# r-barnes/richdem

Measured on NVIDIA H100. Metric: Priority-Flood fill + D8 flow accumulation throughput, higher is better.
Workload: dtype f32

## Files before the change

richdem_b200/csrc/fill.cu:

```cuda
#include "common.cuh"

#include <chrono>

namespace rdb {

namespace {

#ifndef RDB_TX
#define RDB_TX 64
#endif
#ifndef RDB_TY
#define RDB_TY 64
#endif
#ifndef RDB_FILL_THREADS
#define RDB_FILL_THREADS 128
#endif
#ifndef RDB_FILL_MIN_CTAS
#define RDB_FILL_MIN_CTAS 6
#endif
constexpr int TX = RDB_TX;
constexpr int TY = RDB_TY;
constexpr int BXN = TX / 4;
constexpr int BYN = TY / 4;
constexpr int PADL = 4;
constexpr int SP = TX + 2 * PADL;
constexpr int SROWS = TY + 2;
constexpr int FILL_THREADS = RDB_FILL_THREADS;
constexpr int FILL_MIN_CTAS = RDB_FILL_MIN_CTAS;
static_assert(BYN <= 16 && BXN * BYN <= 256 && TX % 4 == 0 && TY % 4 == 0, "tile shape");
constexpr uint32_t W_TILE_BYTES = SP * SROWS * 4;
constexpr uint32_t Z_TILE_BYTES = TX * TY * 4;

struct RoundCtl {
  int count;
  int take;
};

struct FillDev {
  RoundCtl ctl[3];
  RoundCtl proc[3];
  unsigned long long visits;
  unsigned long long iters;
  unsigned long long block_updates;
  unsigned long long warp_updates;
  unsigned long long idle_visits;
  unsigned long long iter_hist[8];
  int edge_changed;
  int zmin_ord, zmax_ord;
  unsigned long long deferred;
  unsigned long long live_rounds;
  float level, step, step_min, level_max;
  int target, ordered;
  int ndefer[3];
};

struct FillArgs {
  const float *Z;
  int zpitch, zox, zoy, zext;
  const float *coarse;
  int Wc, pool, yoff;
  int *staged;
  float *Wp;
  int pitch;
  int W, H;
  int tilesX, tilesY;
  int *list0, *list1;
  int *stamp;
  int *sides;
  int *keys;
  float level;
  int *plist;
  int use_proc;
  FillDev *dev;
  int round;
  int max_iters;
  int use_tma;
  int profile;
  int *dirty;
};

__device__ __forceinline__ uint32_t smem_u32(const void *p) {
  return (uint32_t)__cvta_generic_to_shared(p);
}
__device__ __forceinline__ void mbar_init(unsigned long long *bar, int count) {
  asm volatile("mbarrier.init.shared::cta.b64 [%0], %1;" ::"r"(smem_u32(bar)), "r"(count) : "memory");
}
__device__ __forceinline__ void mbar_arrive_expect_tx(unsigned long long *bar, uint32_t bytes) {
  asm volatile("mbarrier.arrive.expect_tx.shared::cta.b64 _, [%0], %1;" ::"r"(smem_u32(bar)),
               "r"(bytes)
               : "memory");
}
__device__ __forceinline__ void mbar_wait(unsigned long long *bar, uint32_t parity) {
  uint32_t ok;
  const uint32_t addr = smem_u32(bar);
  do {
    asm volatile(
        "{\n"
        "  .reg .pred p;\n"
        "  mbarrier.try_wait.parity.shared::cta.b64 p, [%1], %2;\n"
        "  selp.u32 %0, 1, 0, p;\n"
        "}\n"
        : "=r"(ok)
        : "r"(addr), "r"(parity)
        : "memory");
  } while (!ok);
}
__device__ __forceinline__ void tma_load_2d(void *smem_dst, const CUtensorMap *map, int c0, int c1,
                                            unsigned long long *bar) {
  asm volatile(
      "cp.async.bulk.tensor.2d.shared::cluster.global.mbarrier::complete_tx::bytes [%0], [%1, {%2, %3}], [%4];"
      ::"r"(smem_u32(smem_dst)),
      "l"((unsigned long long)map), "r"(c0), "r"(c1), "r"(smem_u32(bar))
      : "memory");
}
__device__ __forceinline__ void fence_proxy_async() {
  asm volatile("fence.proxy.async.shared::cta;" ::: "memory");
}

constexpr int NBLK = BXN * BYN;
constexpr int MKP = BXN + 2;
constexpr int NWARP = FILL_THREADS / 32;
constexpr int SEG = ((NBLK + NWARP - 1) / NWARP + 31) / 32 * 32;
enum : int { SIDE_N = 1, SIDE_S = 2, SIDE_W = 4, SIDE_E = 8, SIDE_NW = 16, SIDE_NE = 32, SIDE_SW = 64,
             SIDE_SE = 128, SIDE_FULL = 256 };

__host__ __device__ __forceinline__ int f2ord(float f) {
  int b;
  memcpy(&b, &f, 4);
  return b >= 0 ? b : (b ^ 0x7fffffff);
}
__host__ __device__ __forceinline__ float ord2f(int o) {
  const int b = o >= 0 ? o : (o ^ 0x7fffffff);
  float f;
  memcpy(&f, &b, 4);
  return f;
}
constexpr int ORD_POS_INF = 0x7f800000;

__device__ __forceinline__ void enqueue_tile(const FillArgs &a, RoundCtl *next, int *list_next, int t,
                                             int stampval, int side_bits, int key_ord) {
  atomicOr(&a.sides[(stampval & 1) * a.tilesX * a.tilesY + t], side_bits);
  atomicMin(&a.keys[(stampval & 1) * a.tilesX * a.tilesY + t], key_ord);
  if (atomicExch(&a.stamp[t], stampval) != stampval) {
    const int idx = atomicAdd(&next->count, 1);
    list_next[idx] = t;
  }
}

__device__ __forceinline__ float min3f(float a, float b, float c) { return fminf(fminf(a, b), c); }

constexpr bool DRAIN_SWEEPS = TX == 64 && TY == 64 && FILL_THREADS == 128;

template <bool TOPO4>
__device__ __forceinline__ void fill_drain_sweeps(float *sW, const float *sZ, int y0, int H, int *sFlags, int *sKey) {
  const unsigned FULL = 0xffffffffu;
  const int tid = threadIdx.x, lane = tid & 31, wrp = tid >> 5;
  const int x = 32 * (wrp & 1) + lane;
  const bool down = wrp < 2;
  const int dy = down ? 1 : -1;
  const bool ecol = x < 4 || x >= TX - 4;
  unsigned long long rows = 0;
  float kmin = __int_as_float(0x7f800000);
  int y = down ? 0 : TY - 1;
  float p = sW[(y - dy + 1) * SP + PADL + x];
#pragma unroll 1
  for (int half = 0; half < 2; half++) {
#pragma unroll 8
    for (int s = 0; s < TY / 2; s++, y += dy) {
      const float zz = sZ[y * TX + x];
      float *cell = &sW[(y + 1) * SP + PADL + x];
      const float w = *cell;
      float m = p;
      if (!TOPO4) {
        float pl = __shfl_up_sync(FULL, p, 1), pr = __shfl_down_sync(FULL, p, 1);
        const float *prow = &sW[(y - dy + 1) * SP + PADL + x];
        if (lane == 0) pl = prow[-1];
        if (lane == 31) pr = prow[1];
        m = min3f(pl, p, pr);
      }
      const float nw = fminf(w, fmaxf(zz, m));
      p = w;
      if (nw < w) {
        *cell = nw;
        p = nw;
        rows |= 1ull << y;
        if (ecol || y < 4 || y >= TY - 4) kmin = fminf(kmin, nw);
      }
    }
    __syncthreads();
  }
  int f = 0;
#pragma unroll
  for (int by = 0; by < BYN; by++)
    if ((rows >> (4 * by)) & 0xFull) f |= 1 << (12 + by);
  if (rows & 1ull) f |= SIDE_N;
  if (rows >> (TY - 1)) f |= SIDE_S;
  if (x == 0 && rows) f |= SIDE_W | (rows & 1ull ? SIDE_NW : 0) | (rows >> (TY - 1) ? SIDE_SW : 0);
  if (x == TX - 1 && rows) f |= SIDE_E | (rows & 1ull ? SIDE_NE : 0) | (rows >> (TY - 1) ? SIDE_SE : 0);
  const int j1 = 1 - y0, j2 = (H - 2) - y0;
  if (j1 >= 0 && j1 < TY && ((rows >> j1) & 1ull)) f |= 1 << 9;
  if (j2 >= 0 && j2 < TY && ((rows >> j2) & 1ull)) f |= 1 << 10;
#pragma unroll
  for (int o = 16; o > 0; o >>= 1) {
    f |= __shfl_xor_sync(FULL, f, o);
    kmin = fminf(kmin, __shfl_xor_sync(FULL, kmin, o));
  }
  if (lane == 0 && f) {
    atomicOr(sFlags, f);
    if (f & 0xFF) atomicMin(sKey, f2ord(kmin));
  }
}

template <int STEP, bool TOPO4 = false, bool STAGE = false>
__global__ void __launch_bounds__(FILL_THREADS, FILL_MIN_CTAS)
    fill_sweep_kernel(const __grid_constant__ CUtensorMap mapW, const __grid_constant__ CUtensorMap mapZ,
                      const FillArgs a) {
  __shared__ __align__(128) float sW[SROWS * SP];
  __shared__ __align__(128) float sZ[TY * TX];
  __shared__ __align__(8) unsigned long long mbar;
  __shared__ unsigned char sMark[MKP * (BYN + 2)];
  __shared__ unsigned char sList[2][NWARP][SEG];
  __shared__ __align__(16) int sCnt[2][NWARP];
  __shared__ int sTile;
  __shared__ int sFlags;
  __shared__ int sKey;
  __shared__ int sProf[2];
  __shared__ int sNbDone;

  const int tid = threadIdx.x;
  const int r = a.round;
  RoundCtl *cur = &a.dev->ctl[r % 3];
  RoundCtl *next = &a.dev->ctl[(r + 1) % 3];
  const int *list_cur = (r & 1) ? a.list1 : a.list0;
  int *list_next = (r & 1) ? a.list0 : a.list1;
  const int ntiles = a.tilesX * a.tilesY;
  if (a.use_proc) {
    cur = &a.dev->proc[r % 3];
    list_cur = a.plist;
  }
  const int n = cur->count;

  if (blockIdx.x == 0 && tid == 0) {
    RoundCtl *z = &a.dev->ctl[(r + 2) % 3];
    z->count = 0;
    z->take = 0;
    RoundCtl *zp = &a.dev->proc[(r + 1) % 3];
    zp->count = 0;
    zp->take = 0;
    if (n > 0) {
      atomicAdd(&a.dev->visits, (unsigned long long)n);
      a.dev->live_rounds++;
    }
  }
  if (n == 0) return;

  if (tid == 0) {
    mbar_init(&mbar, 1);
    asm volatile("fence.mbarrier_init.release.cluster;" ::: "memory");
  }
  uint32_t phase = 0;
  const int max_iters = a.max_iters;

  for (;;) {
    if (tid == 0) sTile = atomicAdd(&cur->take, 1);
    for (int k = tid; k < MKP * (BYN + 2); k += FILL_THREADS) sMark[k] = 0;
    __syncthreads();
    const int li = sTile;
    if (li >= n) break;
    const int t = list_cur[li];
    const int tyT = t / a.tilesX, txT = t - tyT * a.tilesX;
    const int x0 = txT * TX, y0 = tyT * TY;

    constexpr bool stage = STAGE;
    if (tid == 0) {
      sFlags = 0;
      sKey = ORD_POS_INF;
      sProf[0] = sProf[1] = 0;
      if (stage) {
        int nb = 0;
        for (int dy = -1; dy <= 1; dy++)
          for (int dx = -1; dx <= 1; dx++) {
            const int ty = tyT + dy, tx = txT + dx;
            if ((dx | dy) && ty >= 0 && ty < a.tilesY && tx >= 0 && tx < a.tilesX &&
                *reinterpret_cast<volatile int *>(&a.staged[ty * a.tilesX + tx]))
              nb |= 1 << ((dy + 1) * 3 + dx + 1);
          }
        __threadfence();
        sNbDone = nb;
      }
    }
    if (a.use_tma) {
      if (tid == 0) {
        fence_proxy_async();
        mbar_arrive_expect_tx(&mbar, (stage ? 0u : W_TILE_BYTES) + Z_TILE_BYTES);
        if (!stage) tma_load_2d(sW, &mapW, x0, y0, &mbar);
        tma_load_2d(sZ, &mapZ, x0 + a.zox, y0 + a.zoy, &mbar);
      }
    } else {
      if (!stage) {
        for (int k = tid; k < SROWS * (SP / 4); k += FILL_THREADS) {
          const int rr = k / (SP / 4), cc = k - rr * (SP / 4);
          reinterpret_cast<float4 *>(sW)[k] =
              __ldcg(reinterpret_cast<const float4 *>(a.Wp + (size_t)(y0 + rr) * a.pitch + x0) + cc);
        }
      }
      const float inf = __int_as_float(0x7f800000);
      for (int k = tid; k < TY * (TX / 4); k += FILL_THREADS) {
        const int rr = k / (TX / 4), cc = k - rr * (TX / 4);
        reinterpret_cast<float4 *>(sZ)[k] =
            a.zext && (y0 + rr >= a.H || x0 + 4 * cc >= a.W)
                ? make_float4(inf, inf, inf, inf)
                : __ldg(reinterpret_cast<const float4 *>(a.Z + (size_t)(y0 + a.zoy + rr) * a.zpitch + x0 + a.zox) + cc);
      }
    }
    int sides = a.sides[(r & 1) * ntiles + t];
    __syncthreads();
    if (tid == 0) {
      a.sides[(r & 1) * ntiles + t] = 0;
      a.keys[(r & 1) * ntiles + t] = ORD_POS_INF;
    }
    if (stage) {
      const float inf = __int_as_float(0x7f800000);
      const int nbdone = sNbDone;
      constexpr int C4N = SP / 4, RSTEP = FILL_THREADS / C4N;
      static_assert(RSTEP >= 1, "a CTA covers one row of the window");
      if (tid < RSTEP * C4N) {
        const int c4 = 4 * (tid % C4N);
        int rr = tid / C4N;
        const int dx = c4 < PADL ? -1 : (c4 >= PADL + TX ? 1 : 0);
        const int xb = x0 + c4 - PADL;
        const int cx = xb >= 0 ? xb / a.pool : 0, rx = xb - cx * a.pool;
        const int yy = y0 + rr - 1 + a.yoff;
        int cy = (yy + a.pool) / a.pool - 1, ry = yy - cy * a.pool;
        const int dq = RSTEP / a.pool, dr = RSTEP - dq * a.pool;
        for (; rr < SROWS; rr += RSTEP) {
          const int dy = rr == 0 ? -1 : (rr == SROWS - 1 ? 1 : 0);
          float4 v4;
          if ((nbdone >> ((dy + 1) * 3 + dx + 1)) & 1) {
            v4 = __ldcg(reinterpret_cast<const float4 *>(a.Wp + (size_t)(y0 + rr) * a.pitch + x0 + c4));
          } else {
            const int y = y0 + rr - 1;
            float v[4] = {inf, inf, inf, inf};
            if (y >= 0 && y < a.H) {
              const float *crow = a.coarse + (size_t)cy * a.Wc;
              const float *zrow = a.Z + (size_t)(y + a.zoy) * a.zpitch + a.zox;
              const bool brow = y == 0 || y == a.H - 1;
              const float c0 = (a.pool & 3) == 0 && xb >= 0 && xb < a.W ? __ldg(crow + cx) : inf;
              int cc = cx, rc = rx;
#pragma unroll
              for (int j = 0; j < 4; j++) {
                const int x = xb + j;
                if (j > 0 && ++rc == a.pool) {
                  rc = 0;
                  cc++;
                }
                if (x >= 0 && x < a.W)
                  v[j] = brow || x == 0 || x == a.W - 1 ? __ldg(zrow + x) : (a.pool & 3) == 0 ? c0 : __ldg(crow + cc);
              }
            }
            v4 = make_float4(v[0], v[1], v[2], v[3]);
          }
          *reinterpret_cast<float4 *>(&sW[rr * SP + c4]) = v4;
          cy += dq;
          ry += dr;
          if (ry >= a.pool) {
            ry -= a.pool;
            cy++;
          }
        }
      }
    }
#include "fill_relax_body.inc"

    if (f) {
      atomicOr(&sFlags, f);
      if (f & 0xFF) atomicMin(&sKey, f2ord(kmin));
    }
    __syncthreads();
    const int fl = sFlags;
    const int rowch = (fl >> 12) & 0xFFFF;
    const int rowout = stage ? (1 << BYN) - 1 : rowch;
    if (rowout) {
      for (int k = tid; k < TY * (TX / 4); k += FILL_THREADS) {
        const int rr = k / (TX / 4), cc = k % (TX / 4);
        if (rowout & (1 << (rr >> 2))) {
          const float4 val = *reinterpret_cast<const float4 *>(&sW[(rr + 1) * SP + PADL + 4 * cc]);
          __stcg(reinterpret_cast<float4 *>(a.Wp + (size_t)(y0 + 1 + rr) * a.pitch + (x0 + PADL)) + cc, val);
        }
      }
    }
    if (stage) {
      __syncthreads();
      if (tid == 0) {
        __threadfence();
        atomicExch(&a.staged[t], 1);
      }
    }
    if (rowch) {
      if (tid < 8) {
        const int sv = r + 1;
        const bool n_ok = tyT > 0, s_ok = tyT < a.tilesY - 1, w_ok = txT > 0, e_ok = txT < a.tilesX - 1;
        int nb = -1, bits = 0;
        switch (tid) {
          case 0: if ((fl & SIDE_N) && n_ok) { nb = t - a.tilesX; bits = SIDE_S; } break;
          case 1: if ((fl & SIDE_S) && s_ok) { nb = t + a.tilesX; bits = SIDE_N; } break;
          case 2: if ((fl & SIDE_W) && w_ok) { nb = t - 1; bits = SIDE_E; } break;
          case 3: if ((fl & SIDE_E) && e_ok) { nb = t + 1; bits = SIDE_W; } break;
          case 4: if ((fl & SIDE_NW) && n_ok && w_ok) { nb = t - a.tilesX - 1; bits = SIDE_SE; } break;
          case 5: if ((fl & SIDE_NE) && n_ok && e_ok) { nb = t - a.tilesX + 1; bits = SIDE_SW; } break;
          case 6: if ((fl & SIDE_SW) && s_ok && w_ok) { nb = t + a.tilesX - 1; bits = SIDE_NE; } break;
          default: if ((fl & SIDE_SE) && s_ok && e_ok) { nb = t + a.tilesX + 1; bits = SIDE_NW; } break;
        }
        if (nb >= 0) enqueue_tile(a, next, list_next, nb, sv, bits, sKey);
        if (tid == 0 && (fl & (3 << 9))) atomicOr(&a.dev->edge_changed, (fl >> 9) & 3);
        if (tid == 0 && a.dirty) a.dirty[t] = 1;
      }
    }
    if (tid == 0) {
      if (again) enqueue_tile(a, next, list_next, t, r + 1, SIDE_FULL, f2ord(-__int_as_float(0x7f800000)));
      atomicAdd(&a.dev->iters, (unsigned long long)iters);
      if (a.profile) {
        if (!rowch) atomicAdd(&a.dev->idle_visits, 1ull);
        atomicAdd(&a.dev->block_updates, (unsigned long long)sProf[0]);
        atomicAdd(&a.dev->warp_updates, (unsigned long long)sProf[1]);
        const int hb = iters <= 1 ? 0 : iters <= 2 ? 1 : iters <= 4 ? 2 : iters <= 8 ? 3 : iters <= 16 ? 4 : iters <= 32 ? 5 : iters <= 64 ? 6 : 7;
        atomicAdd(&a.dev->iter_hist[hb], 1ull);
      }
    }
  }
}

__global__ void __launch_bounds__(256) fill_admit_kernel(const FillArgs a) {
  const int r = a.round;
  const RoundCtl *cur = &a.dev->ctl[r % 3];
  RoundCtl *next = &a.dev->ctl[(r + 1) % 3];
  RoundCtl *proc = &a.dev->proc[r % 3];
  const int *list_cur = (r & 1) ? a.list1 : a.list0;
  int *list_next = (r & 1) ? a.list0 : a.list1;
  const int n = cur->count;
  const int ntiles = a.tilesX * a.tilesY;
  const float level = a.level;
  int nd = 0;
  for (int i = blockIdx.x * blockDim.x + threadIdx.x; i < n; i += gridDim.x * blockDim.x) {
    const int t = list_cur[i];
    const int kord = a.keys[(r & 1) * ntiles + t];
    if (ord2f(kord) <= level) {
      a.plist[atomicAdd(&proc->count, 1)] = t;
    } else {
      int bits = a.sides[(r & 1) * ntiles + t];
      if (bits == 0) bits = SIDE_FULL;
      a.sides[(r & 1) * ntiles + t] = 0;
      a.keys[(r & 1) * ntiles + t] = ORD_POS_INF;
      enqueue_tile(a, next, list_next, t, r + 1, bits, kord);
      nd++;
    }
  }
  for (int o = 16; o > 0; o >>= 1) nd += __shfl_xor_sync(0xffffffffu, nd, o);
  if ((threadIdx.x & 31) == 0 && nd) atomicAdd(&a.dev->ndefer[r % 3], nd);
}

__global__ void __launch_bounds__(256) fill_seed_kernel(const FillArgs a, const int *__restrict__ tiles, int n) {
  const int i = blockIdx.x * blockDim.x + threadIdx.x;
  if (i >= n) return;
  const int r = a.round;
  RoundCtl *cur = &a.dev->ctl[r % 3];
  int *list_cur = (r & 1) ? a.list1 : a.list0;
  enqueue_tile(a, cur, list_cur, tiles[i], r, SIDE_FULL, f2ord(-__int_as_float(0x7f800000)));
}

__global__ void __launch_bounds__(256) fill_seed_flags_kernel(const FillArgs a, const int *__restrict__ flag, int ntiles,
                                                               int *count) {
  const int t = blockIdx.x * blockDim.x + threadIdx.x;
  if (t >= ntiles || !flag[t]) return;
  const int r = a.round;
  RoundCtl *cur = &a.dev->ctl[r % 3];
  int *list_cur = (r & 1) ? a.list1 : a.list0;
  enqueue_tile(a, cur, list_cur, t, r, SIDE_FULL, f2ord(-__int_as_float(0x7f800000)));
  if (count) atomicAdd(count, 1);
}

__global__ void __launch_bounds__(256) fill_ghost_update_kernel(float *Wp, float *Zp, int pitch, int W, int H, int y,
                                                                 const float *__restrict__ row, int *tile_flag, int tilesX,
                                                                 int *lowered) {
  const int x = blockIdx.x * blockDim.x + threadIdx.x;
  if (x >= W) return;
  const size_t o = (size_t)(y + 1) * pitch + x + PADL;
  const float v = row[x];
  if (v < Wp[o]) {
    Wp[o] = v;
    Zp[o] = v;
    *lowered = 1;
    const int ya = y > 0 ? y - 1 : 0, yb = y < H - 1 ? y + 1 : H - 1, xa = x > 0 ? x - 1 : 0, xb = x < W - 1 ? x + 1 : W - 1;
    const int ty0 = ya / TY, ty1 = yb / TY, tx0 = xa / TX, tx1 = xb / TX;
    tile_flag[ty0 * tilesX + tx0] = 1;
    if (tx1 != tx0) tile_flag[ty0 * tilesX + tx1] = 1;
    if (ty1 != ty0) {
      tile_flag[ty1 * tilesX + tx0] = 1;
      if (tx1 != tx0) tile_flag[ty1 * tilesX + tx1] = 1;
    }
  }
}

__global__ void __launch_bounds__(256) fill_lift_row_kernel(float *row, int W, const float *__restrict__ coarse_row, int k) {
  const int x = blockIdx.x * blockDim.x + threadIdx.x;
  if (x < W) row[x] = coarse_row[x / k];
}

template <bool LIFT>
__global__ void fill_init_kernel(const float *__restrict__ dem, float *__restrict__ Zp,
                                 float *__restrict__ Wp, int W, int H, int pitch, int rows, FillDev *dev,
                                 const float *__restrict__ coarse, int Wc, int pool, int yoff) {
  const int px4 = (blockIdx.x * blockDim.x + threadIdx.x) * 4;
  const float inf = __int_as_float(0x7f800000);
  float lo = inf, hi = -inf;
  for (int py = blockIdx.y; py < rows && px4 < pitch; py += gridDim.y) {
    float zv[4], wv[4];
    const int y = py - 1;
#pragma unroll
    for (int k = 0; k < 4; k++) {
      const int x = px4 + k - PADL;
      float zz = inf, ww = inf;
      if (x >= 0 && x < W && y >= 0 && y < H) {
        zz = dem[(size_t)y * W + x];
        const bool border = (x == 0) | (y == 0) | (x == W - 1) | (y == H - 1);
        ww = border ? zz : (LIFT ? __ldg(coarse + (size_t)((y + yoff) / pool) * Wc + x / pool) : inf);
        if (zz < inf && zz > -inf) {
          lo = fminf(lo, zz);
          hi = fmaxf(hi, zz);
        }
      }
      zv[k] = zz;
      wv[k] = ww;
    }
    const size_t o = (size_t)py * pitch + px4;
    if (Zp) *reinterpret_cast<float4 *>(Zp + o) = make_float4(zv[0], zv[1], zv[2], zv[3]);
    *reinterpret_cast<float4 *>(Wp + o) = make_float4(wv[0], wv[1], wv[2], wv[3]);
  }
  for (int o = 16; o > 0; o >>= 1) {
    lo = fminf(lo, __shfl_xor_sync(0xffffffffu, lo, o));
    hi = fmaxf(hi, __shfl_xor_sync(0xffffffffu, hi, o));
  }
  __shared__ float slo[4], shi[4];
  if ((threadIdx.x & 31) == 0) {
    slo[threadIdx.x >> 5] = lo;
    shi[threadIdx.x >> 5] = hi;
  }
  __syncthreads();
  if (threadIdx.x == 0) {
    lo = fminf(fminf(slo[0], slo[1]), fminf(slo[2], slo[3]));
    hi = fmaxf(fmaxf(shi[0], shi[1]), fmaxf(shi[2], shi[3]));
    if (lo <= hi) {
      atomicMin(&dev->zmin_ord, f2ord(lo));
      atomicMax(&dev->zmax_ord, f2ord(hi));
    }
  }
}

__global__ void __launch_bounds__(256) fill_frame_kernel(float *__restrict__ Wp, int pitch, int rows) {
  const int i = blockIdx.x * blockDim.x + threadIdx.x;
  const float inf = __int_as_float(0x7f800000);
  if (i < pitch) {
    Wp[i] = inf;
    Wp[(size_t)(rows - 1) * pitch + i] = inf;
  }
  if (i < rows) {
#pragma unroll
    for (int j = 0; j < PADL; j++) {
      Wp[(size_t)i * pitch + j] = inf;
      Wp[(size_t)i * pitch + pitch - PADL + j] = inf;
    }
  }
}

constexpr int HIST_BINS = 1024;
__global__ void __launch_bounds__(256) fill_hist_kernel(const float *__restrict__ Z, int zpitch, int ncols, int nrows,
                                                         int row_stride, float zmin, float inv_range, unsigned int *hist) {
  __shared__ unsigned int sh[HIST_BINS];
  for (int k = threadIdx.x; k < HIST_BINS; k += blockDim.x) sh[k] = 0;
  __syncthreads();
  const int row = blockIdx.x * row_stride;
  if (row < nrows) {
    for (int x = threadIdx.x; x < ncols; x += blockDim.x) {
      const float zv = Z[(size_t)row * zpitch + x];
      if (zv < __int_as_float(0x7f800000) && zv > -__int_as_float(0x7f800000)) {
        int b = (int)((zv - zmin) * inv_range * HIST_BINS);
        b = b < 0 ? 0 : (b >= HIST_BINS ? HIST_BINS - 1 : b);
        atomicAdd(&sh[b], 1u);
      }
    }
  }
  __syncthreads();
  for (int k = threadIdx.x; k < HIST_BINS; k += blockDim.x)
    if (sh[k]) atomicAdd(&hist[k], sh[k]);
}

__global__ void __launch_bounds__(128) dist_pad_init_kernel(const uint8_t *__restrict__ open, int open_bit,
                                                             const float *__restrict__ winit, float *__restrict__ Zp,
                                                             float *__restrict__ Wp, int W, int H, int pitch, int rows,
                                                             int ghost_top, int ghost_bottom, int *tile_flag, int tilesX) {
  const int px = blockIdx.x * blockDim.x + threadIdx.x;
  if (px >= pitch) return;
  const float inf = __int_as_float(0x7f800000);
  for (int py = blockIdx.y; py < rows; py += gridDim.y) {
    const int x = px - PADL, y = py - 1;
    float zz = inf, ww = inf;
    if (x >= 0 && x < W && y >= 0 && y < H) {
      const size_t i = (size_t)y * W + x;
      if (!((ghost_top && y == 0) || (ghost_bottom && y == H - 1))) {
        if (open[i] & open_bit) zz = 0.0f;
        ww = winit[i];
        if (ww < inf) {
          const int ya = y > 0 ? y - 1 : 0, yb = y < H - 1 ? y + 1 : H - 1, xa = x > 0 ? x - 1 : 0, xb = x < W - 1 ? x + 1 : W - 1;
          const int ty0 = ya / TY, ty1 = yb / TY, tx0 = xa / TX, tx1 = xb / TX;
          tile_flag[ty0 * tilesX + tx0] = 1;
          if (tx1 != tx0) tile_flag[ty0 * tilesX + tx1] = 1;
          if (ty1 != ty0) {
            tile_flag[ty1 * tilesX + tx0] = 1;
            if (tx1 != tx0) tile_flag[ty1 * tilesX + tx1] = 1;
          }
        }
      }
    }
    Zp[(size_t)py * pitch + px] = zz;
    Wp[(size_t)py * pitch + px] = ww;
  }
}

__global__ void fill_i32_kernel(int *p, int v, int n) {
  const int i = blockIdx.x * blockDim.x + threadIdx.x;
  if (i < n) p[i] = v;
}

__global__ void __launch_bounds__(256) fill_maxpool_kernel(const float *__restrict__ src, int W, int H, int yoff, float *dst, int Wc,
                                                            int Hc, int k, int combine) {
  const int bx = blockIdx.x * blockDim.x + threadIdx.x;
  if (bx >= Wc) return;
  const int by_lo = yoff / k, by_hi = (yoff + H - 1) / k;
  for (int by = by_lo + blockIdx.y; by <= by_hi && by < Hc; by += gridDim.y) {
    float m = -__int_as_float(0x7f800000);
    const bool vec = (k & 3) == 0 && (W & 3) == 0 && bx * k + k <= W && ((uintptr_t)src & 15) == 0;
    for (int j = 0; j < k; j++) {
      const int y = by * k + j - yoff;
      if (y < 0) continue;
      if (y >= H) break;
      if (vec) {
        const float4 *row = reinterpret_cast<const float4 *>(src + (size_t)y * W + bx * k);
        for (int i = 0; i < k / 4; i++) {
          const float4 q = __ldg(row + i);
          m = fmaxf(fmaxf(m, fmaxf(q.x, q.y)), fmaxf(q.z, q.w));
        }
      } else {
        for (int i = 0; i < k; i++) {
          const int x = bx * k + i;
          if (x < W) m = fmaxf(m, __ldg(src + (size_t)y * W + x));
        }
      }
    }
    float *o = dst + (size_t)by * Wc + bx;
    *o = combine ? fmaxf(*o, m) : m;
  }
}

__global__ void __launch_bounds__(256) fill_restrict_kernel(const float *__restrict__ Wp, int pitch, int W, int H,
                                                             float *Wc, int cpitch, int Wcw, int Hc, int k,
                                                             const int *__restrict__ dirty, int tilesX, int *ctile_flag,
                                                             int ctilesX) {
  const int bx = blockIdx.x * blockDim.x + threadIdx.x;
  if (bx >= Wcw) return;
  for (int by = blockIdx.y; by < Hc; by += gridDim.y) {
    if (dirty && !dirty[((by * k) / TY) * tilesX + (bx * k) / TX]) continue;
    float m = -__int_as_float(0x7f800000);
    if ((k & 3) == 0 && bx * k + k <= W && by * k + k <= H) {
      for (int j = 0; j < k; j++) {
        const float4 *row = reinterpret_cast<const float4 *>(Wp + (size_t)(by * k + j + 1) * pitch + bx * k + PADL);
        for (int i = 0; i < k / 4; i++) {
          const float4 q = __ldcg(row + i);
          m = fmaxf(fmaxf(m, fmaxf(q.x, q.y)), fmaxf(q.z, q.w));
        }
      }
    } else {
      for (int j = 0; j < k; j++) {
        const int y = by * k + j;
        if (y >= H) break;
        for (int i = 0; i < k; i++) {
          const int x = bx * k + i;
          if (x < W) m = fmaxf(m, __ldcg(Wp + (size_t)(y + 1) * pitch + x + PADL));
        }
      }
    }
    float *o = Wc + (size_t)(by + 1) * cpitch + bx + PADL;
    if (m < *o && bx > 0 && by > 0 && bx < Wcw - 1 && by < Hc - 1) {
      *o = m;
      const int ty0 = (by - 1) / TY, ty1 = (by + 1) / TY, tx0 = (bx - 1) / TX, tx1 = (bx + 1) / TX;
      ctile_flag[ty0 * ctilesX + tx0] = 1;
      if (tx1 != tx0) ctile_flag[ty0 * ctilesX + tx1] = 1;
      if (ty1 != ty0) {
        ctile_flag[ty1 * ctilesX + tx0] = 1;
        if (tx1 != tx0) ctile_flag[ty1 * ctilesX + tx1] = 1;
      }
    }
  }
}

__global__ void __launch_bounds__(256) fill_blockmax_kernel(const float *__restrict__ Wp, int pitch, int W, int y_lo, int y_hi,
                                                             int yoff, float *out, int Wcw, int Hc, int k,
                                                             const int *__restrict__ dirty, int tilesX) {
  const int bx = blockIdx.x * blockDim.x + threadIdx.x;
  if (bx >= Wcw) return;
  const int by_lo = (yoff + y_lo) / k, by_hi = (yoff + y_hi - 1) / k;
  for (int by = by_lo + blockIdx.y; by <= by_hi && by < Hc; by += gridDim.y) {
    if (dirty) {
      int l0 = by * k - yoff, l1 = l0 + k - 1;
      l0 = l0 < y_lo ? y_lo : l0;
      l1 = l1 >= y_hi ? y_hi - 1 : l1;
      const int tx = (bx * k) / TX;
      if (!dirty[(l0 / TY) * tilesX + tx] && !dirty[(l1 / TY) * tilesX + tx]) {
        out[(size_t)by * Wcw + bx] = __int_as_float(0x7f800000);
        continue;
      }
    }
    float m = -__int_as_float(0x7f800000);
    for (int j = 0; j < k; j++) {
      const int y = by * k + j - yoff;
      if (y < y_lo) continue;
      if (y >= y_hi) break;
      for (int i = 0; i < k; i++) {
        const int x = bx * k + i;
        if (x < W) m = fmaxf(m, __ldcg(Wp + (size_t)(y + 1) * pitch + x + PADL));
      }
    }
    float *o = out + (size_t)by * Wcw + bx;
    *o = fmaxf(*o, m);
  }
}

__global__ void __launch_bounds__(256) fill_prolong_kernel(float *Wp, int pitch, int W, int H, const float *__restrict__ Wc,
                                                            int cpitch, int coff_x, int coff_y, int k, int *tile_flag,
                                                            int tilesX, int yoff, const int *__restrict__ cdirty,
                                                            int ctilesX) {
  const int t = blockIdx.x;
  const int tyT = t / tilesX, txT = t - tyT * tilesX;
  const int x0 = txT * TX, y0 = tyT * TY;
  if (cdirty) {
    const int cx0 = (x0 / k) / TX, cx1 = ((x0 + TX - 1) / k) / TX;
    const int cy0 = ((y0 + yoff) / k) / TY, cy1 = ((y0 + TY - 1 + yoff) / k) / TY;
    bool any = false;
    for (int cy = cy0; cy <= cy1; cy++)
      for (int cx = cx0; cx <= cx1; cx++) any |= cdirty[cy * ctilesX + cx] != 0;
    if (!any) return;
  }
  bool lowered = false, lo_n = false, lo_s = false, lo_w = false, lo_e = false;
  for (int g = threadIdx.x; g < TX * TY / 4; g += blockDim.x) {
    const int ly = g / (TX / 4), lx4 = (g - ly * (TX / 4)) * 4;
    const int y = y0 + ly;
    if (y < 1 || y >= H - 1) continue;
    float4 *wp4 = reinterpret_cast<float4 *>(Wp + (size_t)(y + 1) * pitch + x0 + lx4 + PADL);
    const float4 w4 = *wp4;
    float wv[4] = {w4.x, w4.y, w4.z, w4.w};
    const float *crow = Wc + (size_t)((y + yoff) / k + coff_y) * cpitch + coff_x;
    bool any = false;
#pragma unroll
    for (int j = 0; j < 4; j++) {
      const int lx = lx4 + j, x = x0 + lx;
      if (x < 1 || x >= W - 1) continue;
      const float l = __ldg(crow + x / k);
      if (l < wv[j]) {
        wv[j] = l;
        any = true;
        lo_w |= lx == 0;
        lo_e |= lx == TX - 1;
      }
    }
    if (any) {
      *wp4 = make_float4(wv[0], wv[1], wv[2], wv[3]);
      lowered = true;
      lo_n |= ly == 0;
      lo_s |= ly == TY - 1;
    }
  }
  if (lowered) {
    const int tilesY = (H + TY - 1) / TY;
    tile_flag[t] = 1;
    const bool n_ok = tyT > 0, s_ok = tyT < tilesY - 1, w_ok = txT > 0, e_ok = txT < tilesX - 1;
    if (lo_n && n_ok) tile_flag[t - tilesX] = 1;
    if (lo_s && s_ok) tile_flag[t + tilesX] = 1;
    if (lo_w && w_ok) tile_flag[t - 1] = 1;
    if (lo_e && e_ok) tile_flag[t + 1] = 1;
    if (lo_n && lo_w && n_ok && w_ok) tile_flag[t - tilesX - 1] = 1;
    if (lo_n && lo_e && n_ok && e_ok) tile_flag[t - tilesX + 1] = 1;
    if (lo_s && lo_w && s_ok && w_ok) tile_flag[t + tilesX - 1] = 1;
    if (lo_s && lo_e && s_ok && e_ok) tile_flag[t + tilesX + 1] = 1;
  }
}

__global__ void __launch_bounds__(256) fill_finish_x4_kernel(const float *__restrict__ Wp, float *__restrict__ out, int W,
                                                              int H, int pitch) {
  const int x4 = (blockIdx.x * blockDim.x + threadIdx.x) * 4;
  if (x4 >= W) return;
  for (int y = blockIdx.y; y < H; y += gridDim.y) {
    const float4 v = __ldcs(reinterpret_cast<const float4 *>(Wp + (size_t)(y + 1) * pitch + x4 + PADL));
    __stcs(reinterpret_cast<float4 *>(out + (size_t)y * W + x4), v);
  }
}

__global__ void fill_finish_kernel(const float *__restrict__ Wp, float *__restrict__ out, int W, int H,
                                   int pitch) {
  const int x = blockIdx.x * blockDim.x + threadIdx.x;
  if (x >= W) return;
  for (int y = blockIdx.y; y < H; y += gridDim.y) out[(size_t)y * W + x] = Wp[(size_t)(y + 1) * pitch + x + PADL];
}

typedef CUresult (*EncodeTiledFn)(CUtensorMap *, CUtensorMapDataType, cuuint32_t, void *, const cuuint64_t *,
                                  const cuuint64_t *, const cuuint32_t *, const cuuint32_t *,
                                  CUtensorMapInterleave, CUtensorMapSwizzle, CUtensorMapL2promotion,
                                  CUtensorMapFloatOOBfill);

EncodeTiledFn get_encode_fn() {
  static EncodeTiledFn fn = nullptr;
  if (!fn) {
    void *p = nullptr;
    cudaDriverEntryPointQueryResult q;
    RDB_CK(cudaGetDriverEntryPoint("cuTensorMapEncodeTiled", &p, cudaEnableDefault, &q));
    if (!p || q != cudaDriverEntryPointSuccess) fail("cuTensorMapEncodeTiled not available from the driver");
    fn = (EncodeTiledFn)p;
  }
  return fn;
}

CUtensorMap make_map(float *base, int pitch, int rows, int boxw, int boxh) {
  CUtensorMap m;
  const cuuint64_t gdim[2] = {(cuuint64_t)pitch, (cuuint64_t)rows};
  const cuuint64_t gstride[1] = {(cuuint64_t)pitch * 4};
  const cuuint32_t box[2] = {(cuuint32_t)boxw, (cuuint32_t)boxh};
  const cuuint32_t estr[2] = {1, 1};
  CUresult rc = get_encode_fn()(&m, CU_TENSOR_MAP_DATA_TYPE_FLOAT32, 2, base, gdim, gstride, box, estr,
                                CU_TENSOR_MAP_INTERLEAVE_NONE, CU_TENSOR_MAP_SWIZZLE_NONE,
                                CU_TENSOR_MAP_L2_PROMOTION_L2_128B, CU_TENSOR_MAP_FLOAT_OOB_FILL_NONE);
  if (rc != CUDA_SUCCESS) fail("cuTensorMapEncodeTiled failed with CUresult %d", (int)rc);
  return m;
}

}

struct FillState {
  int W = 0, H = 0, pitch = 0, rows = 0, tilesX = 0, tilesY = 0;
  DevBuf<float> Zp, Wp;
  DevBuf<int> list0, list1, plist, stamp, sides, keys;
  DevBuf<int> dirty, tflag;
  DevBuf<int> staged;
  float zmin = 0.f, zmax = 0.f;
  bool first_run = true;
  bool ordered = false;
  int step_mode = 0;
  bool topo4 = false;
  std::vector<float> levels;
  DevBuf<FillDev> dev;
  CUtensorMap mapW, mapZ;
  int round = 0;
  int grid = 0;
  int64_t rounds_run = 0;
  int64_t live_rounds = 0;
  int64_t visits_seen = 0;
  bool still_active = false;
  int64_t sched_round = 0;

  const float *zext = nullptr;
  const float *stage_coarse = nullptr;
  int stage_wc = 0, stage_k = 1, stage_yoff = 0;

  void begin(const float *d_dem, int w, int h, const float *d_coarse = nullptr, int coarse_w = 0, int coarse_k = 0,
             int coarse_yoff = 0, bool dem_stays = false) {
    Ctx &c = ctx();
    W = w;
    H = h;
    tilesX = (w + TX - 1) / TX;
    tilesY = (h + TY - 1) / TY;
    pitch = tilesX * TX + 2 * PADL;
    rows = tilesY * TY + 2;
    const size_t np = (size_t)pitch * rows;
    zext = dem_stays && c.params.fill_external_z != 0 && (w & 3) == 0 && ((uintptr_t)d_dem & 15) == 0 ? d_dem : nullptr;
    stage_coarse = zext && d_coarse ? d_coarse : nullptr;
    stage_wc = coarse_w;
    stage_k = coarse_k;
    stage_yoff = coarse_yoff;
    if (zext) Zp.reset();
    else Zp.alloc(np);
    Wp.alloc(np);
    const size_t nt = (size_t)tilesX * tilesY;
    list0.alloc(nt);
    list1.alloc(nt);
    plist.alloc(nt);
    stamp.alloc(nt);
    sides.alloc(2 * nt);
    keys.alloc(2 * nt);
    dev.alloc(1);
    RDB_CK(cudaMemsetAsync(stamp.p, 0, nt * sizeof(int), c.stream));
    RDB_CK(cudaMemsetAsync(sides.p, 0, 2 * nt * sizeof(int), c.stream));
    if (stage_coarse) {
      staged.alloc(nt);
      RDB_CK(cudaMemsetAsync(staged.p, 0, nt * sizeof(int), c.stream));
    }
    {
      FillDev h0;
      memset(&h0, 0, sizeof(h0));
      h0.zmin_ord = ORD_POS_INF;
      h0.zmax_ord = f2ord(-__builtin_inff());
      memcpy(c.pinned, &h0, sizeof(h0));
      RDB_CK(cudaMemcpyAsync(dev.p, c.pinned, sizeof(FillDev), cudaMemcpyHostToDevice, c.stream));
    }
    {
      const int n2 = (int)(2 * nt);
      fill_i32_kernel<<<(n2 + 255) / 256, 256, 0, c.stream>>>(keys.p, ORD_POS_INF, n2);
      dim3 blk(128), grd((pitch / 4 + 127) / 128, rows < 2048 ? rows : 2048);
      if (stage_coarse) {
        const int n = pitch > rows ? pitch : rows;
        fill_frame_kernel<<<(n + 255) / 256, 256, 0, c.stream>>>(Wp.p, pitch, rows);
      } else if (d_coarse) {
        fill_init_kernel<true><<<grd, blk, 0, c.stream>>>(d_dem, Zp.p, Wp.p, W, H, pitch, rows, dev.p, d_coarse, coarse_w, coarse_k,
                                                         coarse_yoff);
      } else {
        fill_init_kernel<false><<<grd, blk, 0, c.stream>>>(d_dem, Zp.p, Wp.p, W, H, pitch, rows, dev.p, nullptr, 0, 1, 0);
      }
      RDB_CK(cudaGetLastError());
      count_launch(2);
      zmin = zmax = 0.f;
      if (!d_coarse) {
        FillDev *hd = (FillDev *)c.pinned;
        RDB_CK(cudaMemcpyAsync(hd, dev.p, sizeof(FillDev), cudaMemcpyDeviceToHost, c.stream));
        RDB_CK(cudaStreamSynchronize(c.stream));
        zmin = ord2f(hd->zmin_ord);
        zmax = ord2f(hd->zmax_ord);
        if (!(zmin <= zmax)) zmin = zmax = 0.f;
      }
      ordered = c.params.fill_ordered != 0 && zmax > zmin && !d_coarse;
      levels.clear();
      if (ordered) {
        int64_t R = c.params.fill_order_rounds;
        if (R <= 0) R = (int64_t)(0.8 * (tilesX > tilesY ? tilesX : tilesY));
        if (R < 8) {
          ordered = false;
        } else {
          DevBuf<unsigned int> hist(HIST_BINS);
          RDB_CK(cudaMemsetAsync(hist.p, 0, HIST_BINS * sizeof(unsigned int), c.stream));
          const int stride = rows > 4096 ? 16 : (rows > 512 ? 4 : 1);
          const int nb = (rows - 2 + stride - 1) / stride;
          if (zext)
            fill_hist_kernel<<<nb, 256, 0, c.stream>>>(zext, W, W, H, stride, zmin, 1.0f / (zmax - zmin), hist.p);
          else
            fill_hist_kernel<<<nb, 256, 0, c.stream>>>(Zp.p + pitch, pitch, pitch, rows - 1, stride, zmin, 1.0f / (zmax - zmin),
                                                       hist.p);
          RDB_CK(cudaGetLastError());
          count_launch();
          unsigned int *hh = (unsigned int *)c.pinned;
          RDB_CK(cudaMemcpyAsync(hh, hist.p, HIST_BINS * sizeof(unsigned int), cudaMemcpyDeviceToHost, c.stream));
          RDB_CK(cudaStreamSynchronize(c.stream));
          double total = 0;
          for (int k = 0; k < HIST_BINS; k++) total += hh[k];
          levels.resize((size_t)R);
          double cum = 0;
          int bin = 0;
          for (int64_t k = 0; k < R; k++) {
            const double want = total * (double)(k + 1) / (double)R;
            while (bin < HIST_BINS - 1 && cum + hh[bin] < want) cum += hh[bin++];
            levels[(size_t)k] = zmin + (zmax - zmin) * (float)(bin + 1) / (float)HIST_BINS;
          }
        }
      }
    }
    mapW = make_map(Wp.p, pitch, rows, SP, SROWS);
    mapZ = zext ? make_map(const_cast<float *>(zext), W, H, TX, TY) : make_map(Zp.p, pitch, rows, TX, TY);
    int per_sm = 0;
    RDB_CK(cudaOccupancyMaxActiveBlocksPerMultiprocessor(&per_sm, fill_sweep_kernel<0>, FILL_THREADS, 0));
    if (per_sm < 1) per_sm = 1;
    grid = c.num_sms * per_sm;
    round = 1;
    std::vector<int> init;
    for (int ty = 0; ty < tilesY; ty++)
      for (int tx = 0; tx < tilesX; tx++)
        if (d_coarse || ty == 0 || tx == 0 || ty == tilesY - 1 || tx == tilesX - 1) init.push_back(ty * tilesX + tx);
    seed_worklist(init);
  }

  void begin_dist(const uint8_t *d_open, int open_bit, const float *d_winit, int w, int h, int ghost_top = 0,
                  int ghost_bottom = 0) {
    Ctx &c = ctx();
    step_mode = 1;
    W = w;
    H = h;
    tilesX = (w + TX - 1) / TX;
    tilesY = (h + TY - 1) / TY;
    pitch = tilesX * TX + 2 * PADL;
    rows = tilesY * TY + 2;
    const size_t np = (size_t)pitch * rows;
    Zp.alloc(np);
    Wp.alloc(np);
    const size_t nt = (size_t)tilesX * tilesY;
    list0.alloc(nt);
    list1.alloc(nt);
    plist.alloc(nt);
    stamp.alloc(nt);
    sides.alloc(2 * nt);
    keys.alloc(2 * nt);
    dev.alloc(1);
    RDB_CK(cudaMemsetAsync(stamp.p, 0, nt * sizeof(int), c.stream));
    RDB_CK(cudaMemsetAsync(sides.p, 0, 2 * nt * sizeof(int), c.stream));
    RDB_CK(cudaMemsetAsync(dev.p, 0, sizeof(FillDev), c.stream));
    const int n2 = (int)(2 * nt);
    fill_i32_kernel<<<(n2 + 255) / 256, 256, 0, c.stream>>>(keys.p, ORD_POS_INF, n2);
    dim3 blk(128), grd((pitch + 127) / 128, rows < 2048 ? rows : 2048);
    clear_flags();
    dist_pad_init_kernel<<<grd, blk, 0, c.stream>>>(d_open, open_bit, d_winit, Zp.p, Wp.p, W, H, pitch, rows, ghost_top,
                                                    ghost_bottom, tflag.p, tilesX);
    RDB_CK(cudaGetLastError());
    count_launch(2);
    ordered = false;
    mapW = make_map(Wp.p, pitch, rows, SP, SROWS);
    mapZ = make_map(Zp.p, pitch, rows, TX, TY);
    int per_sm = 0;
    RDB_CK(cudaOccupancyMaxActiveBlocksPerMultiprocessor(&per_sm, fill_sweep_kernel<1>, FILL_THREADS, 0));
    if (per_sm < 1) per_sm = 1;
    grid = c.num_sms * per_sm;
    round = 1;
    seed_from_flags();
  }

  void seed_worklist(const std::vector<int> &tiles) {
    Ctx &c = ctx();
    if (tiles.empty()) return;
    DevBuf<int> d(tiles.size());
    RDB_CK(cudaMemcpyAsync(d.p, tiles.data(), tiles.size() * sizeof(int), cudaMemcpyHostToDevice, c.stream));
    FillArgs a = make_args();
    a.round = round;
    fill_seed_kernel<<<(unsigned)((tiles.size() + 255) / 256), 256, 0, c.stream>>>(a, d.p, (int)tiles.size());
    RDB_CK(cudaGetLastError());
    count_launch();
    RDB_CK(cudaStreamSynchronize(c.stream));
  }

  FillArgs make_args() {
    Ctx &c = ctx();
    FillArgs a;
    memset(&a, 0, sizeof(a));
    if (zext) {
      a.Z = zext;
      a.zpitch = W;
      a.zext = 1;
    } else {
      a.Z = Zp.p;
      a.zpitch = pitch;
      a.zox = PADL;
      a.zoy = 1;
    }
    a.Wc = stage_wc;
    a.pool = stage_k;
    a.yoff = stage_yoff;
    a.staged = staged.p;
    a.Wp = Wp.p;
    a.pitch = pitch;
    a.W = W;
    a.H = H;
    a.tilesX = tilesX;
    a.tilesY = tilesY;
    a.list0 = list0.p;
    a.list1 = list1.p;
    a.stamp = stamp.p;
    a.sides = sides.p;
    a.keys = keys.p;
    a.plist = plist.p;
    a.dev = dev.p;
    a.max_iters = (int)c.params.fill_max_iters;
    a.use_tma = (int)c.params.fill_use_tma;
    a.profile = (int)c.params.fill_profile;
    a.level = __builtin_inff();
    a.dirty = dirty.p;
    return a;
  }

  bool timed = true;
  int batch_edge = 0;
  void launch_batch(int per_sync) {
    Ctx &c = ctx();
    FillArgs a = make_args();
    if (timed) RDB_CK(cudaEventRecord(c.evk0, c.stream));
    for (int k = 0; k < per_sync; k++) {
      a.round = round;
      if (ordered && sched_round < (int64_t)levels.size()) {
        a.level = levels[(size_t)sched_round];
        a.use_proc = 1;
        fill_admit_kernel<<<c.num_sms * 2, 256, 0, c.stream>>>(a);
        c.stats.kernel_launches++;
      } else {
        a.level = __builtin_inff();
        a.use_proc = 0;
      }
      sched_round++;
      a.coarse = round == 1 ? stage_coarse : nullptr;
      if (step_mode) fill_sweep_kernel<1><<<grid, FILL_THREADS, 0, c.stream>>>(mapW, mapZ, a);
      else if (a.coarse && topo4) fill_sweep_kernel<0, true, true><<<grid, FILL_THREADS, 0, c.stream>>>(mapW, mapZ, a);
      else if (a.coarse) fill_sweep_kernel<0, false, true><<<grid, FILL_THREADS, 0, c.stream>>>(mapW, mapZ, a);
      else if (topo4) fill_sweep_kernel<0, true><<<grid, FILL_THREADS, 0, c.stream>>>(mapW, mapZ, a);
      else fill_sweep_kernel<0><<<grid, FILL_THREADS, 0, c.stream>>>(mapW, mapZ, a);
      round++;
    }
    if (timed) RDB_CK(cudaEventRecord(c.evk1, c.stream));
    RDB_CK(cudaGetLastError());
    RDB_CK(cudaMemcpyAsync(c.pinned, dev.p, sizeof(FillDev), cudaMemcpyDeviceToHost, c.stream));
    c.stats.kernel_launches += per_sync;
    rounds_run += per_sync;
    if (round > (1 << 30)) fail("fill: round counter overflow");
  }
  bool collect() {
    Ctx &c = ctx();
    RDB_CK(cudaStreamSynchronize(c.stream));
    if (timed) {
      float t = 0;
      RDB_CK(cudaEventElapsedTime(&t, c.evk0, c.evk1));
      c.stats.ms_main_kernel += t;
    }
    const FillDev *hd = (const FillDev *)c.pinned;
    still_active = hd->ctl[round % 3].count != 0;
    if (!still_active) first_run = false;
    live_rounds = (int64_t)hd->live_rounds;
    visits_seen = (int64_t)hd->visits;
    iters_seen = (int64_t)hd->iters;
    batch_edge = hd->edge_changed;
    return still_active;
  }
  int64_t iters_seen = 0;

  int run(int64_t max_rounds = 0) {
    Ctx &c = ctx();
    int64_t rounds_this_call = 0;
    int per_sync = (int)(c.params.fill_rounds_per_sync > 0 ? c.params.fill_rounds_per_sync : 16);
    if (max_rounds > 0 && max_rounds < per_sync) per_sync = (int)max_rounds;
    RDB_CK(cudaMemsetAsync(&dev.p->edge_changed, 0, sizeof(int), c.stream));
    for (;;) {
      launch_batch(per_sync);
      collect();
      rounds_this_call += per_sync;
      if (!still_active) break;
      if (max_rounds > 0 && rounds_this_call >= max_rounds) break;
    }
    const FillDev *hd = (const FillDev *)c.pinned;
    c.stats.fill_rounds = live_rounds;
    c.stats.fill_tile_visits = visits_seen;
    c.stats.fill_tile_iters = iters_seen;
    c.stats.fill_tile_cells = TX * TY;
    if (c.params.fill_profile) {
      fprintf(stderr, "[fill profile] deferred=%llu visits=%llu iters=%llu block_updates=%llu (%.1f%% of 256/iter) warp_updates=%llu (%.1f%% of 8/iter) idle_visits=%llu hist(1,2,3-4,5-8,9-16,17-32,33-64,65+)=",
              hd->deferred, hd->visits, hd->iters, hd->block_updates, 100.0 * hd->block_updates / (256.0 * hd->iters + 1),
              hd->warp_updates, 100.0 * hd->warp_updates / (8.0 * hd->iters + 1), hd->idle_visits);
      for (int k = 0; k < 8; k++) fprintf(stderr, "%llu ", hd->iter_hist[k]);
      fprintf(stderr, "\n");
    }
    return batch_edge | (still_active ? 4 : 0);
  }

  void track_dirty() {
    Ctx &c = ctx();
    const size_t nt = (size_t)tilesX * tilesY;
    dirty.alloc(nt);
    RDB_CK(cudaMemsetAsync(dirty.p, 0, nt * sizeof(int), c.stream));
  }
  void clear_dirty() {
    if (dirty.p) RDB_CK(cudaMemsetAsync(dirty.p, 0, (size_t)tilesX * tilesY * sizeof(int), ctx().stream));
  }
  void seed_from_flags(int *d_count = nullptr) {
    Ctx &c = ctx();
    const int nt = tilesX * tilesY;
    FillArgs a = make_args();
    a.round = round;
    fill_seed_flags_kernel<<<(nt + 255) / 256, 256, 0, c.stream>>>(a, tflag.p, nt, d_count);
    RDB_CK(cudaGetLastError());
    count_launch();
  }
  void clear_flags() {
    const size_t nt = (size_t)tilesX * tilesY;
    if (!tflag.p) tflag.alloc(nt);
    RDB_CK(cudaMemsetAsync(tflag.p, 0, nt * sizeof(int), ctx().stream));
  }
  void restrict_into(FillState &cs, int k) {
    Ctx &c = ctx();
    cs.clear_flags();
    const bool selective = dirty.p && TX % k == 0 && TY % k == 0;
    dim3 blk(256), grd((unsigned)((cs.W + 255) / 256), (unsigned)(cs.H < 4096 ? cs.H : 4096));
    fill_restrict_kernel<<<grd, blk, 0, c.stream>>>(Wp.p, pitch, W, H, cs.Wp.p, cs.pitch, cs.W, cs.H, k,
                                                    selective ? dirty.p : nullptr, tilesX, cs.tflag.p, cs.tilesX);
    RDB_CK(cudaGetLastError());
    count_launch();
    cs.seed_from_flags();
    clear_dirty();
  }
  void blockmax_into(float *d_out, int wc, int hc, int k, int yoff, int y_lo, int y_hi, bool selective = false) {
    Ctx &c = ctx();
    dim3 blk(256), grd((unsigned)((wc + 255) / 256), (unsigned)((y_hi - y_lo) / k + 2 < 4096 ? (y_hi - y_lo) / k + 2 : 4096));
    const bool sel = selective && dirty.p && TX % k == 0;
    fill_blockmax_kernel<<<grd, blk, 0, c.stream>>>(Wp.p, pitch, W, y_lo, y_hi, yoff, d_out, wc, hc, k, sel ? dirty.p : nullptr, tilesX);
    RDB_CK(cudaGetLastError());
    count_launch();
    if (sel) clear_dirty();
  }
  void prolong_from(const float *d_wc, int cpitch, int coff_x, int coff_y, int k, int yoff = 0, const int *cdirty = nullptr,
                    int ctilesX = 0, int *d_count = nullptr) {
    Ctx &c = ctx();
    clear_flags();
    const int nt = tilesX * tilesY;
    fill_prolong_kernel<<<nt, 256, 0, c.stream>>>(Wp.p, pitch, W, H, d_wc, cpitch, coff_x, coff_y, k, tflag.p, tilesX, yoff,
                                                  cdirty, ctilesX);
    RDB_CK(cudaGetLastError());
    count_launch();
    seed_from_flags(d_count);
  }
  void prolong_from_level(FillState &cs, int k, int yoff = 0, int *d_count = nullptr) {
    prolong_from(cs.Wp.p, cs.pitch, PADL, 1, k, yoff, cs.dirty.p, cs.tilesX, d_count);
    cs.clear_dirty();
  }
  void ghost_update(int y, const float *d_row, int *d_lowered) {
    Ctx &c = ctx();
    clear_flags();
    fill_ghost_update_kernel<<<(W + 255) / 256, 256, 0, c.stream>>>(Wp.p, Zp.p, pitch, W, H, y, d_row, tflag.p, tilesX, d_lowered);
    RDB_CK(cudaGetLastError());
    count_launch();
    seed_from_flags();
  }

  void read_row(int y, float *d_row) {
    if (y < 0 || y >= H) fail("fill_read_row: row %d out of range", y);
    RDB_CK(cudaMemcpyAsync(d_row, Wp.p + (size_t)(y + 1) * pitch + PADL, (size_t)W * 4,
                           cudaMemcpyDeviceToDevice, ctx().stream));
  }

  void update_row(int y, const float *d_row) {
    if (y != 0 && y != H - 1) fail("fill_update_row: only boundary rows (0, height-1) can be replaced");
    Ctx &c = ctx();
    const size_t o = (size_t)(y + 1) * pitch + PADL;
    RDB_CK(cudaMemcpyAsync(Wp.p + o, d_row, (size_t)W * 4, cudaMemcpyDeviceToDevice, c.stream));
    RDB_CK(cudaMemcpyAsync(Zp.p + o, d_row, (size_t)W * 4, cudaMemcpyDeviceToDevice, c.stream));
    pending_rows.push_back(y);
  }
  std::vector<int> pending_rows;

  void activate_pending() {
    if (pending_rows.empty()) return;
    std::vector<char> mark((size_t)tilesX * tilesY, 0);
    std::vector<int> tiles;
    for (int y : pending_rows) {
      for (int yy = y - 1; yy <= y + 1; yy++) {
        if (yy < 0 || yy >= H) continue;
        const int tyT = yy / TY;
        for (int tx = 0; tx < tilesX; tx++) {
          const int t = tyT * tilesX + tx;
          if (!mark[t]) {
            mark[t] = 1;
            tiles.push_back(t);
          }
        }
      }
    }
    pending_rows.clear();
    seed_worklist(tiles);
  }

  void finish(float *d_out) {
    Ctx &c = ctx();
    if ((W & 3) == 0 && ((uintptr_t)d_out & 15) == 0) {
      dim3 blk(256), grd((W / 4 + 255) / 256, H < 4096 ? H : 4096);
      fill_finish_x4_kernel<<<grd, blk, 0, c.stream>>>(Wp.p, d_out, W, H, pitch);
    } else {
      dim3 blk(256), grd((W + 255) / 256, H < 32768 ? H : 32768);
      fill_finish_kernel<<<grd, blk, 0, c.stream>>>(Wp.p, d_out, W, H, pitch);
    }
    RDB_CK(cudaGetLastError());
    count_launch();
  }
};

void geodesic_distance_dev(const uint8_t *d_open, int open_bit, float *d_w_inout, int w, int h) {
  Ctx &c = ctx();
  FillState st;
  const rdb200_stats saved = c.stats;
  st.begin_dist(d_open, open_bit, d_w_inout, w, h);
  st.run();
  st.finish(d_w_inout);
  RDB_CK(cudaStreamSynchronize(c.stream));
  const int64_t launches = c.stats.kernel_launches;
  const int64_t rounds = c.stats.fill_rounds;
  c.stats = saved;
  c.stats.kernel_launches = launches;
  c.stats.flat_bfs_levels += rounds;
}

void geodesic_distance_pair_dev(const uint8_t *d_open, int open_bit, float *d_wa, float *d_wb, int w, int h) {
  Ctx &c = ctx();
  if (!c.aux_stream[0]) {
    RDB_CK(cudaStreamCreateWithFlags(&c.aux_stream[0], cudaStreamNonBlocking));
    RDB_CK(cudaStreamCreateWithFlags(&c.aux_stream[1], cudaStreamNonBlocking));
    RDB_CK(cudaEventCreateWithFlags(&c.aux_event[0], cudaEventDisableTiming));
    RDB_CK(cudaEventCreateWithFlags(&c.aux_event[1], cudaEventDisableTiming));
    RDB_CK(cudaEventCreateWithFlags(&c.aux_event[2], cudaEventDisableTiming));
  }
  const rdb200_stats saved = c.stats;
  cudaStream_t main_stream = c.stream;
  void *main_pinned = c.pinned;
  RDB_CK(cudaEventRecord(c.aux_event[2], main_stream));
  FillState st[2];
  float *wbuf[2] = {d_wa, d_wb};
  auto lane = [&](int k, auto &&fn) {
    c.stream = c.aux_stream[k];
    c.pinned = (char *)main_pinned + 8192 * (k + 1);
    try {
      fn(st[k]);
    } catch (...) {
      c.stream = main_stream;
      c.pinned = main_pinned;
      throw;
    }
    c.stream = main_stream;
    c.pinned = main_pinned;
  };
  static_assert(sizeof(FillDev) <= 8192, "pinned slot");
  try {
    for (int k = 0; k < 2; k++) {
      RDB_CK(cudaStreamWaitEvent(c.aux_stream[k], c.aux_event[2], 0));
      lane(k, [&](FillState &s) {
        s.timed = false;
        s.begin_dist(d_open, open_bit, wbuf[k], w, h);
        s.grid = s.grid > 1 ? s.grid / 2 : 1;
      });
    }
    const int per_sync = (int)(c.params.fill_rounds_per_sync > 0 ? c.params.fill_rounds_per_sync : 16);
    bool live[2] = {true, true};
    while (live[0] || live[1]) {
      for (int k = 0; k < 2; k++)
        if (live[k]) lane(k, [&](FillState &s) { s.launch_batch(per_sync); });
      for (int k = 0; k < 2; k++)
        if (live[k]) lane(k, [&](FillState &s) { live[k] = s.collect(); });
    }
    for (int k = 0; k < 2; k++) {
      lane(k, [&](FillState &s) { s.finish(wbuf[k]); });
      RDB_CK(cudaEventRecord(c.aux_event[k], c.aux_stream[k]));
      RDB_CK(cudaStreamWaitEvent(main_stream, c.aux_event[k], 0));
    }
  } catch (...) {
    cudaStreamSynchronize(c.aux_stream[0]);
    cudaStreamSynchronize(c.aux_stream[1]);
    throw;
  }
  RDB_CK(cudaStreamSynchronize(c.aux_stream[0]));
  RDB_CK(cudaStreamSynchronize(c.aux_stream[1]));
  const int64_t launches = c.stats.kernel_launches;
  c.stats = saved;
  c.stats.kernel_launches = launches;
  c.stats.flat_bfs_levels += st[0].live_rounds + st[1].live_rounds;
}

static void fill_depressions_level(float *d_dem, int w, int h, int depth, bool topo4 = false) {
  Ctx &c = ctx();
  const int k = (int)c.params.fill_multigrid;
  const int min_side = (int)(c.params.fill_multigrid_min > 0 ? c.params.fill_multigrid_min : 1024);
  FillState st;
  st.topo4 = topo4;
  if (k >= 2 && depth < 8 && w >= min_side && h >= min_side && w / k >= 3 && h / k >= 3) {
    const int wc = (w + k - 1) / k, hc = (h + k - 1) / k;
    DevBuf<float> coarse((size_t)wc * hc);
    dim3 blk(256), grd((unsigned)((wc + 255) / 256), (unsigned)(hc < 4096 ? hc : 4096));
    fill_maxpool_kernel<<<grd, blk, 0, c.stream>>>(d_dem, w, h, 0, coarse.p, wc, hc, k, 0);
    RDB_CK(cudaGetLastError());
    count_launch();
    const int every = (int)c.params.fill_vcycle;
    DevBuf<float> zc;
    if (every > 0) {
      zc.alloc((size_t)wc * hc);
      RDB_CK(cudaMemcpyAsync(zc.p, coarse.p, (size_t)wc * hc * sizeof(float), cudaMemcpyDeviceToDevice, c.stream));
    }
    const rdb200_stats before = c.stats;
    fill_depressions_level(coarse.p, wc, hc, depth + 1, topo4);
    rdb200_stats extra = c.stats;
    extra.fill_rounds -= before.fill_rounds;
    extra.fill_tile_visits -= before.fill_tile_visits;
    extra.fill_tile_iters -= before.fill_tile_iters;
    st.begin(d_dem, w, h, coarse.p, wc, k, 0, true);
    if (every <= 0) {
      st.run();
    } else {
      FillState cst;
      cst.topo4 = topo4;
      cst.begin(zc.p, wc, hc, coarse.p, wc, 1, 0, true);
      cst.run();
      cst.track_dirty();
      st.track_dirty();
      int64_t coarse_visits0 = c.stats.fill_tile_visits, coarse_iters0 = c.stats.fill_tile_iters;
      const bool trace = c.params.fill_trace != 0;
      auto now_ms = [&]() {
        RDB_CK(cudaStreamSynchronize(c.stream));
        return std::chrono::duration<double, std::milli>(std::chrono::steady_clock::now().time_since_epoch()).count();
      };
      for (int cycle = 0;; cycle++) {
        const double t0 = trace ? now_ms() : 0;
        const int64_t v0 = st.visits_seen, r0 = st.live_rounds;
        const bool active = (st.run(every) & 4) != 0;
        const double t1 = trace ? now_ms() : 0;
        if (trace)
          fprintf(stderr, "[fill trace] depth %d cycle %d: fine run %.3f ms (%lld live rounds, %lld visits)%s\n", depth, cycle,
                  t1 - t0, (long long)(st.live_rounds - r0), (long long)(st.visits_seen - v0), active ? "" : " -> converged");
        if (!active) break;
        if (cycle >= 1000) {
          st.run();
          break;
        }
        st.restrict_into(cst, k);
        const double t2 = trace ? now_ms() : 0;
        const int64_t cv0 = cst.visits_seen, cr0 = cst.live_rounds;
        cst.run();
        const double t3 = trace ? now_ms() : 0;
        st.prolong_from_level(cst, k);
        if (trace) {
          const double t4 = now_ms();
          fprintf(stderr, "[fill trace] depth %d cycle %d: restrict %.3f ms, coarse run %.3f ms (%lld live rounds, %lld visits), "
                          "prolong %.3f ms\n", depth, cycle, t2 - t1, t3 - t2, (long long)(cst.live_rounds - cr0),
                  (long long)(cst.visits_seen - cv0), t4 - t3);
        }
      }
      cst.run(1);
      extra.fill_rounds += cst.live_rounds;
      extra.fill_tile_visits += c.stats.fill_tile_visits;
      extra.fill_tile_iters += c.stats.fill_tile_iters;
      (void)coarse_visits0;
      (void)coarse_iters0;
      st.run(1);
    }
    st.finish(d_dem);
    RDB_CK(cudaStreamSynchronize(c.stream));
    c.stats.fill_rounds = st.live_rounds + extra.fill_rounds;
    c.stats.fill_tile_visits += extra.fill_tile_visits;
    c.stats.fill_tile_iters += extra.fill_tile_iters;
    return;
  }
  if (w <= 2 || h <= 2) return;
  st.begin(d_dem, w, h, nullptr, 0, 0, 0, true);
  st.run();
  st.finish(d_dem);
  RDB_CK(cudaStreamSynchronize(c.stream));
}

void fill_relax_from_dev(const float *d_dem, float *d_w, int w, int h) {
  Ctx &c = ctx();
  c.stats.cells = (int64_t)w * h;
  if (w <= 2 || h <= 2) {
    RDB_CK(cudaMemcpyAsync(d_w, d_dem, (size_t)w * h * sizeof(float), cudaMemcpyDeviceToDevice, c.stream));
    RDB_CK(cudaStreamSynchronize(c.stream));
    return;
  }
  FillState st;
  st.begin(d_dem, w, h, d_w, w, 1);
  st.run();
  st.finish(d_w);
  RDB_CK(cudaStreamSynchronize(c.stream));
}

void fill_maxpool_rows(const float *d_src, int w, int h, int yoff, float *d_coarse, int wc, int hc, int k, dim3 grd, dim3 blk) {
  fill_maxpool_kernel<<<grd, blk, 0, ctx().stream>>>(d_src, w, h, yoff, d_coarse, wc, hc, k, 1);
  RDB_CK(cudaGetLastError());
  count_launch();
}

void mgpu_fill_band(const rdb200_comm *comm, float *d_local, int w, int hloc, int gt, int gb, int row0, int H, int *xrounds,
                    bool topo4) {
  Ctx &c = ctx();
  const int world = comm_world(comm);
  gt = gt ? 1 : 0;
  gb = gb ? 1 : 0;
  if (w < 3 || hloc - gt - gb < 1 || hloc < 3) fail("mgpu_fill: band too small (%d x %d)", w, hloc);
  if (row0 < 0 || row0 + hloc > H) fail("mgpu_fill: rows [%d, %d) are outside the raster (%d rows)", row0, row0 + hloc, H);
  int k = (int)c.params.fill_band_multigrid;
  if (k <= 0) {
    k = (int)c.params.fill_multigrid;
    if (k >= 2 && world > 2 && TX % (2 * k) == 0) k *= 2;
  }
  const int min_side = (int)(c.params.fill_multigrid_min > 0 ? c.params.fill_multigrid_min : 1024);
  const bool mg = k >= 2 && w >= min_side && H >= min_side && w / k >= 3 && H / k >= 3 && c.params.fill_multigrid >= 2;
  const int R = (int)(c.params.fill_vcycle > 0 ? c.params.fill_vcycle : 8);
  const float inf = __builtin_inff();
  DevBuf<float> rows(4 * (size_t)w);
  DevBuf<int> flags(4);
  float *send_up = rows.p, *send_dn = rows.p + w, *recv_up = rows.p + 2 * (size_t)w, *recv_dn = rows.p + 3 * (size_t)w;
  FillState st, cst;
  DevBuf<float> zc, wcoarse, bm;
  int wc = 0, hc = 0;
  auto fill_f32 = [&](float *p, size_t n, float v) {
    int bits;
    memcpy(&bits, &v, 4);
    fill_i32_kernel<<<(unsigned)((n + 255) / 256), 256, 0, c.stream>>>(reinterpret_cast<int *>(p), bits, (int)n);
    RDB_CK(cudaGetLastError());
  };
  const bool trace0 = c.params.fill_trace != 0;
  double t0_prev = 0;
  auto lap0 = [&](const char *what) {
    if (!trace0) return;
    RDB_CK(cudaStreamSynchronize(c.stream));
    const double t = std::chrono::duration<double, std::milli>(std::chrono::steady_clock::now().time_since_epoch()).count();
    if (what) fprintf(stderr, "[mgpu fill trace] rank %d begin: %-32s %8.3f ms\n", comm_rank(comm), what, t - t0_prev);
    t0_prev = t;
  };
  lap0(nullptr);
  if (mg) {
    wc = (w + k - 1) / k;
    hc = (H + k - 1) / k;
    const size_t nc = (size_t)wc * hc;
    zc.alloc(nc);
    wcoarse.alloc(nc);
    bm.alloc(nc);
    fill_f32(zc.p, nc, -inf);
    {
      const int hown = hloc - gt - gb;
      dim3 blk(256), grd((unsigned)((wc + 255) / 256), (unsigned)(hown / k + 2 < 4096 ? hown / k + 2 : 4096));
      fill_maxpool_rows(d_local + (size_t)gt * w, w, hown, row0 + gt, zc.p, wc, hc, k, grd, blk);
    }
    lap0("max-pool own rows");
    comm_allreduce(comm, zc.p, nc, RDB200_MAX_F32);
    lap0("all-reduce pooled raster");
    RDB_CK(cudaMemcpyAsync(wcoarse.p, zc.p, nc * sizeof(float), cudaMemcpyDeviceToDevice, c.stream));
    fill_depressions_level(wcoarse.p, wc, hc, 1, topo4);
    lap0("coarse fill (replicated)");
    for (int side = 0; side < 2; side++) {
      if (!(side == 0 ? gt : gb)) continue;
      const int y = side == 0 ? 0 : hloc - 1;
      fill_lift_row_kernel<<<(w + 255) / 256, 256, 0, c.stream>>>(d_local + (size_t)y * w, w, wcoarse.p + (size_t)((row0 + y) / k) * wc, k);
    }
    RDB_CK(cudaGetLastError());
    st.topo4 = topo4;
    st.begin(d_local, w, hloc, wcoarse.p, wc, k, row0);
    lap0("band start (lifted)");
    cst.topo4 = topo4;
    cst.begin(zc.p, wc, hc, wcoarse.p, wc, 1);
    cst.run();
    cst.track_dirty();
    st.track_dirty();
    lap0("coarse solver setup");
  } else {
    if (gt) fill_f32(d_local, (size_t)w, inf);
    if (gb) fill_f32(d_local + (size_t)(hloc - 1) * w, (size_t)w, inf);
    st.topo4 = topo4;
    st.begin(d_local, w, hloc);
  }
  int cycles = 0;
  bool vcycle_on = true;
  int *hflags = (int *)c.pinned + 1024;
  const bool trace = c.params.fill_trace != 0;
  double t_prev = 0;
  auto lap = [&](const char *what) {
    if (!trace) return;
    RDB_CK(cudaStreamSynchronize(c.stream));
    const double t = std::chrono::duration<double, std::milli>(std::chrono::steady_clock::now().time_since_epoch()).count();
    if (what) fprintf(stderr, "[mgpu fill trace] rank %d cycle %d: %-28s %8.3f ms\n", comm_rank(comm), cycles, what, t - t_prev);
    t_prev = t;
  };
  lap(nullptr);
  for (;; cycles++) {
    if (cycles > 100000) fail("mgpu_fill: no convergence");
    const bool active = (st.run(world > 1 || mg ? R : 0) & 4) != 0;
    lap("band sweeps");
    RDB_CK(cudaMemsetAsync(flags.p, 0, 4 * sizeof(int), c.stream));
    if (world > 1) {
      if (gt) st.read_row(1, send_up);
      if (gb) st.read_row(hloc - 2, send_dn);
      comm_exchange(comm, send_up, recv_up, send_dn, recv_dn, (size_t)w * sizeof(float));
      if (gt) st.ghost_update(0, recv_up, flags.p + 1);
      if (gb) st.ghost_update(hloc - 1, recv_dn, flags.p + 1);
      lap("halo exchange");
    }
    if (mg && vcycle_on) {
      fill_f32(bm.p, (size_t)wc * hc, -inf);
      st.blockmax_into(bm.p, wc, hc, k, row0, gt, hloc - gb, true);
      lap("block maxima");
      comm_allreduce(comm, bm.p, (size_t)wc * hc, RDB200_MAX_F32);
      lap("all-reduce coarse");
      cst.prolong_from(bm.p, wc, 0, 0, 1, 0, nullptr, 0, flags.p + 2);
      cst.run();
      lap("coarse relaxation");
      st.prolong_from_level(cst, k, row0, flags.p + 3);
      lap("prolongation");
    }
    if (active) fill_i32_kernel<<<1, 1, 0, c.stream>>>(flags.p, 1, 1);
    comm_allreduce(comm, flags.p, 4, RDB200_MAX_I32);
    RDB_CK(cudaMemcpyAsync(hflags, flags.p, 4 * sizeof(int), cudaMemcpyDeviceToHost, c.stream));
    RDB_CK(cudaStreamSynchronize(c.stream));
    lap("termination vote");
    if (!(hflags[0] | hflags[1] | hflags[2] | hflags[3])) break;
    const int few = st.tilesX * st.tilesY / 64 > 32 ? st.tilesX * st.tilesY / 64 : 32;
    if (trace) fprintf(stderr, "[mgpu fill trace] rank %d cycle %d: flags active=%d ghost=%d coarse=%d fine=%d (cut-off %d)\n",
                       comm_rank(comm), cycles, hflags[0], hflags[1], hflags[2], hflags[3], few);
    if (hflags[2] + hflags[3] < few) vcycle_on = false;
  }
  st.run(1);
  const int64_t visits = st.visits_seen, iters = st.iters_seen, rounds = st.live_rounds;
  st.finish(d_local);
  RDB_CK(cudaStreamSynchronize(c.stream));
  lap("finish");
  c.stats.fill_rounds = rounds + (mg ? cst.live_rounds : 0);
  c.stats.fill_tile_visits = visits;
  c.stats.fill_tile_iters = iters;
  c.stats.fill_tile_cells = TX * TY;
  if (xrounds) *xrounds = cycles + 1;
}

void fill_depressions_dev(float *d_dem, int w, int h, bool topo4) {
  Ctx &c = ctx();
  c.stats.cells = (int64_t)w * h;
  if (w <= 2 || h <= 2) return;
  fill_depressions_level(d_dem, w, h, 0, topo4);
}

}

struct rdb200_fill_state {
  rdb::FillState st;
};

namespace rdb {
rdb200_fill_state *new_band_distance_state(const uint8_t *d_open, int open_bit, const float *d_winit, int w, int h,
                                           int ghost_top, int ghost_bottom) {
  auto *s = new rdb200_fill_state();
  try {
    s->st.begin_dist(d_open, open_bit, d_winit, w, h, ghost_top, ghost_bottom);
  } catch (...) {
    delete s;
    throw;
  }
  return s;
}
void finish_band_distance_state(rdb200_fill_state *s, float *d_out) {
  s->st.finish(d_out);
  RDB_CK(cudaStreamSynchronize(ctx().stream));
  delete s;
}

int mgpu_relax_band(const rdb200_comm *comm, rdb200_fill_state *state, int gt, int gb, int R) {
  Ctx &c = ctx();
  FillState &st = state->st;
  const int world = comm_world(comm), w = st.W, h = st.H;
  DevBuf<float> rows(4 * (size_t)w);
  DevBuf<int> flags(2);
  float *send_up = rows.p, *send_dn = rows.p + w, *recv_up = rows.p + 2 * (size_t)w, *recv_dn = rows.p + 3 * (size_t)w;
  int *hflags = (int *)c.pinned + 1024;
  for (int cycles = 1;; cycles++) {
    if (cycles > 100000) fail("mgpu_relax_band: no convergence");
    const bool active = (st.run(world > 1 ? R : 0) & 4) != 0;
    if (world == 1) {
      if (active) continue;
      RDB_CK(cudaStreamSynchronize(c.stream));
      return cycles;
    }
    RDB_CK(cudaMemsetAsync(flags.p, 0, 2 * sizeof(int), c.stream));
    if (gt) st.read_row(1, send_up);
    if (gb) st.read_row(h - 2, send_dn);
    comm_exchange(comm, send_up, recv_up, send_dn, recv_dn, (size_t)w * sizeof(float));
    if (gt) st.ghost_update(0, recv_up, flags.p + 1);
    if (gb) st.ghost_update(h - 1, recv_dn, flags.p + 1);
    if (active) fill_i32_kernel<<<1, 1, 0, c.stream>>>(flags.p, 1, 1);
    comm_allreduce(comm, flags.p, 2, RDB200_MAX_I32);
    RDB_CK(cudaMemcpyAsync(hflags, flags.p, 2 * sizeof(int), cudaMemcpyDeviceToHost, c.stream));
    RDB_CK(cudaStreamSynchronize(c.stream));
    if (!(hflags[0] | hflags[1])) return cycles;
  }
}
}

namespace rdb {
void capi_set_error(const char *msg);
}

#define RDB_CAPI_TRY try {
#define RDB_CAPI_END                 \
  }                                  \
  catch (const std::exception &e) {  \
    rdb::capi_set_error(e.what());   \
    return 1;                        \
  }                                  \
  return 0;

extern "C" {

int rdb200_dev_fill_begin(rdb200_fill_state **state, const float *d_dem, int32_t width, int32_t height) {
  RDB_CAPI_TRY
  rdb::ensure_init();
  if (!state) rdb::fail("fill_begin: null state pointer");
  if (width < 3 || height < 3) rdb::fail("fill_begin: band must be at least 3x3");
  auto *s = new rdb200_fill_state();
  try {
    s->st.begin(d_dem, width, height);
  } catch (...) {
    delete s;
    throw;
  }
  *state = s;
  RDB_CAPI_END
}

int rdb200_dev_fill_begin_lifted(rdb200_fill_state **state, const float *d_dem, int32_t width, int32_t height,
                                 const float *d_coarse, int32_t coarse_width, int32_t pool, int32_t row_offset) {
  RDB_CAPI_TRY
  rdb::ensure_init();
  if (!state) rdb::fail("fill_begin_lifted: null state pointer");
  if (width < 3 || height < 3) rdb::fail("fill_begin_lifted: band must be at least 3x3");
  if (!d_coarse || pool < 2 || coarse_width < (width + pool - 1) / pool || row_offset < 0)
    rdb::fail("fill_begin_lifted: bad coarse raster (pool %d, coarse_width %d, row_offset %d)", pool, coarse_width, row_offset);
  auto *s = new rdb200_fill_state();
  try {
    s->st.begin(d_dem, width, height, d_coarse, coarse_width, pool, row_offset);
  } catch (...) {
    delete s;
    throw;
  }
  *state = s;
  RDB_CAPI_END
}

int rdb200_dev_maxpool_rows_f32(const float *d_src, int32_t width, int32_t height, int32_t row_offset, int32_t pool,
                                float *d_coarse, int32_t coarse_width, int32_t coarse_height) {
  RDB_CAPI_TRY
  rdb::ensure_init();
  if (width < 1 || height < 1 || pool < 2 || row_offset < 0 || coarse_width < (width + pool - 1) / pool ||
      coarse_height < (row_offset + height + pool - 1) / pool)
    rdb::fail("maxpool_rows: bad geometry");
  rdb::Ctx &c = rdb::ctx();
  dim3 blk(256), grd((unsigned)((coarse_width + 255) / 256), (unsigned)(height / pool + 2 < 4096 ? height / pool + 2 : 4096));
  rdb::fill_maxpool_rows(d_src, width, height, row_offset, d_coarse, coarse_width, coarse_height, pool, grd, blk);
  RDB_CK(cudaStreamSynchronize(c.stream));
  RDB_CAPI_END
}

int rdb200_dev_fill_relax_from_f32(const float *d_dem, float *d_w_inout, int32_t width, int32_t height) {
  RDB_CAPI_TRY
  rdb::ensure_init();
  if (width < 1 || height < 1) rdb::fail("fill_relax_from: raster dimensions must be positive");
  rdb::fill_relax_from_dev(d_dem, d_w_inout, width, height);
  RDB_CAPI_END
}

int rdb200_dev_fill_blockmax(rdb200_fill_state *state, float *d_blockmax, int32_t coarse_width, int32_t coarse_height, int32_t pool,
                             int32_t row_offset, int32_t skip_top, int32_t skip_bottom) {
  RDB_CAPI_TRY
  if (!state) rdb::fail("fill_blockmax: null state");
  rdb::FillState &st = state->st;
  if (pool < 2 || row_offset < 0 || skip_top < 0 || skip_bottom < 0 || skip_top + skip_bottom >= st.H ||
      coarse_width < (st.W + pool - 1) / pool || coarse_height < (row_offset + st.H - skip_bottom + pool - 1) / pool)
    rdb::fail("fill_blockmax: bad geometry");
  st.blockmax_into(d_blockmax, coarse_width, coarse_height, pool, row_offset, skip_top, st.H - skip_bottom);
  RDB_CK(cudaStreamSynchronize(rdb::ctx().stream));
  RDB_CAPI_END
}

int rdb200_dev_fill_prolong(rdb200_fill_state *state, const float *d_coarse, int32_t coarse_width, int32_t pool, int32_t row_offset,
                            int32_t *tiles_lowered) {
  RDB_CAPI_TRY
  if (!state) rdb::fail("fill_prolong: null state");
  if (!d_coarse || pool < 2 || row_offset < 0) rdb::fail("fill_prolong: bad arguments");
  rdb::Ctx &c = rdb::ctx();
  rdb::DevBuf<int> cnt(1);
  RDB_CK(cudaMemsetAsync(cnt.p, 0, sizeof(int), c.stream));
  state->st.prolong_from(d_coarse, coarse_width, 0, 0, pool, row_offset, nullptr, 0, cnt.p);
  int *h = (int *)c.pinned;
  RDB_CK(cudaMemcpyAsync(h, cnt.p, sizeof(int), cudaMemcpyDeviceToHost, c.stream));
  RDB_CK(cudaStreamSynchronize(c.stream));
  if (tiles_lowered) *tiles_lowered = *h;
  RDB_CAPI_END
}

int rdb200_dev_fill_run(rdb200_fill_state *state, int32_t *changed_rows) {
  RDB_CAPI_TRY
  if (!state) rdb::fail("fill_run: null state");
  state->st.activate_pending();
  const int ch = state->st.run(rdb::ctx().params.fill_band_rounds);
  if (changed_rows) *changed_rows = ch;
  RDB_CAPI_END
}

int rdb200_dev_fill_read_row(rdb200_fill_state *state, int32_t y, float *d_row) {
  RDB_CAPI_TRY
  if (!state) rdb::fail("fill_read_row: null state");
  state->st.read_row(y, d_row);
  RDB_CK(cudaStreamSynchronize(rdb::ctx().stream));
  RDB_CAPI_END
}

int rdb200_dev_fill_update_row(rdb200_fill_state *state, int32_t y, const float *d_row) {
  RDB_CAPI_TRY
  if (!state) rdb::fail("fill_update_row: null state");
  state->st.update_row(y, d_row);
  RDB_CK(cudaStreamSynchronize(rdb::ctx().stream));
  RDB_CAPI_END
}

int rdb200_dev_fill_finish(rdb200_fill_state *state, float *d_out) {
  RDB_CAPI_TRY
  if (!state) rdb::fail("fill_finish: null state");
  if (d_out) {
    state->st.finish(d_out);
    RDB_CK(cudaStreamSynchronize(rdb::ctx().stream));
  }
  delete state;
  RDB_CAPI_END
}

}
```

richdem_b200/csrc/fill_relax_body.inc:

```
    if (sides == 0) sides = SIDE_FULL;
    const int lane = tid & 31, wrp = tid >> 5;
    {
      int cntw = 0;
#pragma unroll
      for (int q = 0; q < SEG / 32; q++) {
        const int b = wrp * SEG + 32 * q + lane;
        const int bx = b % BXN, by = b / BXN;
        bool on = (sides & SIDE_FULL) != 0;
        on |= (sides & SIDE_N) && by == 0;
        on |= (sides & SIDE_S) && by == BYN - 1;
        on |= (sides & SIDE_W) && bx == 0;
        on |= (sides & SIDE_E) && bx == BXN - 1;
        on |= (sides & SIDE_NW) && b == 0;
        on |= (sides & SIDE_NE) && b == BXN - 1;
        on |= (sides & SIDE_SW) && b == NBLK - BXN;
        on |= (sides & SIDE_SE) && b == NBLK - 1;
        on &= b < NBLK;
        const unsigned bal = __ballot_sync(0xffffffffu, on);
        if (on) sList[0][wrp][cntw + __popc(bal & ((1u << lane) - 1u))] = (unsigned char)b;
        cntw += __popc(bal);
      }
      if (lane == 0) sCnt[0][wrp] = cntw;
    }
    if (a.use_tma) {
      mbar_wait(&mbar, phase);
      phase ^= 1;
      if (a.zext && (x0 + TX > a.W || y0 + TY > a.H)) {
        for (int k = tid; k < TX * TY; k += FILL_THREADS) {
          const int rr = k / TX, cc = k - rr * TX;
          if (y0 + rr >= a.H || x0 + cc >= a.W) sZ[k] = __int_as_float(0x7f800000);
        }
      }
    }
    __syncthreads();
    if constexpr (STAGE && DRAIN_SWEEPS) fill_drain_sweeps<TOPO4>(sW, sZ, y0, a.H, &sFlags, &sKey);

    int f = 0;
    float kmin = __int_as_float(0x7f800000);
    int iters = 0;
    int cl = 0;
    bool again = false;
    int segn[NWARP];
    int nlist = 0;
#pragma unroll
    for (int w2 = 0; w2 < NWARP; w2++) {
      segn[w2] = sCnt[0][w2];
      nlist += segn[w2];
    }
    while (nlist > 0) {
      for (int i = tid; i < nlist; i += FILL_THREADS) {
        int seg = 0, off = i;
#pragma unroll
        for (int w2 = 0; w2 < NWARP - 1; w2++) {
          if (seg == w2 && off >= segn[w2]) {
            off -= segn[w2];
            seg = w2 + 1;
          }
        }
        const int b = sList[cl][seg][off];
        const int bx = b % BXN, by = b / BXN;
        const int srow = 4 * by + 1, scol = 4 * bx + PADL;
        float v[6][6];
        float z[4][4];
        bool at_floor = true;
#pragma unroll
        for (int j = 0; j < 4; j++) {
          const float4 z4 = *reinterpret_cast<const float4 *>(&sZ[(4 * by + j) * TX + 4 * bx]);
          const float4 m4 = *reinterpret_cast<const float4 *>(&sW[(srow + j) * SP + scol]);
          z[j][0] = z4.x; z[j][1] = z4.y; z[j][2] = z4.z; z[j][3] = z4.w;
          v[j + 1][1] = m4.x; v[j + 1][2] = m4.y; v[j + 1][3] = m4.z; v[j + 1][4] = m4.w;
          at_floor &= (z4.x == m4.x) & (z4.y == m4.y) & (z4.z == m4.z) & (z4.w == m4.w);
        }
        if (at_floor) continue;
#pragma unroll
        for (int j = 0; j < 6; j++) {
          const float *row = &sW[(srow - 1 + j) * SP + scol];
          if (j == 0 || j == 5) {
            const float4 m4 = *reinterpret_cast<const float4 *>(row);
            v[j][1] = m4.x; v[j][2] = m4.y; v[j][3] = m4.z; v[j][4] = m4.w;
          }
          v[j][0] = row[-1];
          v[j][5] = row[4];
        }
        uint32_t ch = 0;
#pragma unroll
        for (int j = 1; j <= 4; j++) {
#pragma unroll
          for (int i2 = 1; i2 <= 4; i2++) {
            const float zz = z[j - 1][i2 - 1];
            const float others = TOPO4 ? min3f(v[j - 1][i2], v[j + 1][i2], v[j][i2 + 1])
                                       : min3f(min3f(v[j - 1][i2 - 1], v[j - 1][i2], v[j - 1][i2 + 1]),
                                               min3f(v[j + 1][i2 - 1], v[j + 1][i2], v[j + 1][i2 + 1]), v[j][i2 + 1]);
            const float b0 = fminf(v[j][i2], fmaxf(zz, STEP ? others + 1.0f : others));
            const float nw = fminf(b0, fmaxf(zz, STEP ? v[j][i2 - 1] + 1.0f : v[j][i2 - 1]));
            if (nw < v[j][i2]) ch |= 1u << ((j - 1) * 4 + (i2 - 1));
            v[j][i2] = nw;
          }
        }
#pragma unroll
        for (int j = 4; j >= 1; j--) {
#pragma unroll
          for (int i2 = 4; i2 >= 1; i2--) {
            const float zz = z[j - 1][i2 - 1];
            const float others = TOPO4 ? min3f(v[j - 1][i2], v[j + 1][i2], v[j][i2 - 1])
                                       : min3f(min3f(v[j - 1][i2 - 1], v[j - 1][i2], v[j - 1][i2 + 1]),
                                               min3f(v[j + 1][i2 - 1], v[j + 1][i2], v[j + 1][i2 + 1]), v[j][i2 - 1]);
            const float b0 = fminf(v[j][i2], fmaxf(zz, STEP ? others + 1.0f : others));
            const float nw = fminf(b0, fmaxf(zz, STEP ? v[j][i2 + 1] + 1.0f : v[j][i2 + 1]));
            if (nw < v[j][i2]) ch |= 1u << ((j - 1) * 4 + (i2 - 1));
            v[j][i2] = nw;
          }
        }
        if (ch) {
#pragma unroll
          for (int j = 0; j < 4; j++) {
            if (ch & (0xFu << (4 * j))) {
              *reinterpret_cast<float4 *>(&sW[(srow + j) * SP + scol]) =
                  make_float4(v[j + 1][1], v[j + 1][2], v[j + 1][3], v[j + 1][4]);
            }
          }
          unsigned char *mk = &sMark[(by + 1) * MKP + (bx + 1)];
          mk[0] = 1;
          if (ch & 0x000Fu) mk[-MKP] = 1;
          if (ch & 0xF000u) mk[MKP] = 1;
          if (ch & 0x1111u) mk[-1] = 1;
          if (ch & 0x8888u) mk[1] = 1;
          if (ch & 0x0001u) mk[-MKP - 1] = 1;
          if (ch & 0x0008u) mk[-MKP + 1] = 1;
          if (ch & 0x1000u) mk[MKP - 1] = 1;
          if (ch & 0x8000u) mk[MKP + 1] = 1;
          if (by == 0 && (ch & 0x000Fu)) f |= SIDE_N;
          if (by == BYN - 1 && (ch & 0xF000u)) f |= SIDE_S;
          if (bx == 0 && (ch & 0x1111u)) f |= SIDE_W;
          if (bx == BXN - 1 && (ch & 0x8888u)) f |= SIDE_E;
          if (b == 0 && (ch & 0x0001u)) f |= SIDE_NW;
          if (b == BXN - 1 && (ch & 0x0008u)) f |= SIDE_NE;
          if (b == NBLK - BXN && (ch & 0x1000u)) f |= SIDE_SW;
          if (b == NBLK - 1 && (ch & 0x8000u)) f |= SIDE_SE;
          {
            const int gy0 = y0 + 4 * by;
            const int j1 = 1 - gy0, j2 = (a.H - 2) - gy0;
            if (j1 >= 0 && j1 < 4 && (ch & (0xFu << (4 * j1)))) f |= 1 << 9;
            if (j2 >= 0 && j2 < 4 && (ch & (0xFu << (4 * j2)))) f |= 1 << 10;
          }
          f |= 1 << (12 + by);
          if (bx == 0 || by == 0 || bx == BXN - 1 || by == BYN - 1) {
#pragma unroll
            for (int j = 0; j < 4; j++)
#pragma unroll
              for (int i2 = 0; i2 < 4; i2++)
                if (ch & (1u << (4 * j + i2))) kmin = fminf(kmin, v[j + 1][i2 + 1]);
          }
        }
      }
      if (a.profile && tid == 0) {
        sProf[0] += nlist;
        sProf[1] += (nlist + 31) / 32;
      }
      iters++;
      __syncthreads();
      {
        int cntw = 0;
#pragma unroll
        for (int q = 0; q < SEG / 32; q++) {
          const int b = wrp * SEG + 32 * q + lane;
          const int mi = (b / BXN + 1) * MKP + (b % BXN) + 1;
          const bool on = (b < NBLK) && sMark[mi] != 0;
          if (on) sMark[mi] = 0;
          const unsigned bal = __ballot_sync(0xffffffffu, on);
          if (on) sList[cl ^ 1][wrp][cntw + __popc(bal & ((1u << lane) - 1u))] = (unsigned char)b;
          cntw += __popc(bal);
        }
        if (lane == 0) sCnt[cl ^ 1][wrp] = cntw;
      }
      __syncthreads();
      cl ^= 1;
      nlist = 0;
#pragma unroll
      for (int w2 = 0; w2 < NWARP; w2++) {
        segn[w2] = sCnt[cl][w2];
        nlist += segn[w2];
      }
      if (nlist > 0 && max_iters > 0 && iters >= max_iters) {
        again = true;
        break;
      }
    }
```

Before: 20360.

## Run fill in place on the DEM buffer with an unpadded layout

Adds an in-place mode in which the water-level grid lives directly in the input DEM buffer with zero offsets. During the staged first round, elevations are copied out to a separate Z buffer via TMA store, or via plain stores when TMA is off. This drops the padded Zp/Wp allocations, the frame kernel and the final copy-out, saving memory traffic and allocation. In exchange, padding has to be emulated with explicit inf masking at tile borders, and every kernel now takes offset parameters.

```diff
diff --git a/richdem_b200/csrc/fill.cu b/richdem_b200/csrc/fill.cu
--- a/richdem_b200/csrc/fill.cu
+++ b/richdem_b200/csrc/fill.cu
@@ -56,12 +56,15 @@
 
 struct FillArgs {
   const float *Z;
-  int zpitch, zox, zoy, zext;
+  int zpitch, zox, zoy;
+  int inplace;
   const float *coarse;
   int Wc, pool, yoff;
   int *staged;
+  float *zcopy;
   float *Wp;
   int pitch;
+  int wox, woy;
   int W, H;
   int tilesX, tilesY;
   int *list0, *list1;
@@ -116,6 +119,14 @@
 __device__ __forceinline__ void fence_proxy_async() {
   asm volatile("fence.proxy.async.shared::cta;" ::: "memory");
 }
+__device__ __forceinline__ void tma_store_2d(const CUtensorMap *map, int c0, int c1, const void *smem_src) {
+  asm volatile("cp.async.bulk.tensor.2d.global.shared::cta.bulk_group [%0, {%1, %2}], [%3];" ::"l"((unsigned long long)map),
+               "r"(c0), "r"(c1), "r"(smem_u32(smem_src))
+               : "memory");
+  asm volatile("cp.async.bulk.commit_group;" ::: "memory");
+}
+__device__ __forceinline__ void bulk_wait_read() { asm volatile("cp.async.bulk.wait_group.read 0;" ::: "memory"); }
+__device__ __forceinline__ void bulk_wait_all() { asm volatile("cp.async.bulk.wait_group 0;" ::: "memory"); }
 
 constexpr int NBLK = BXN * BYN;
 constexpr int MKP = BXN + 2;
@@ -214,7 +225,7 @@
 template <int STEP, bool TOPO4 = false, bool STAGE = false>
 __global__ void __launch_bounds__(FILL_THREADS, FILL_MIN_CTAS)
     fill_sweep_kernel(const __grid_constant__ CUtensorMap mapW, const __grid_constant__ CUtensorMap mapZ,
-                      const FillArgs a) {
+                      const __grid_constant__ CUtensorMap mapZout, const FillArgs a) {
   __shared__ __align__(128) float sW[SROWS * SP];
   __shared__ __align__(128) float sZ[TY * TX];
   __shared__ __align__(8) unsigned long long mbar;
@@ -292,23 +303,27 @@
     if (a.use_tma) {
       if (tid == 0) {
         fence_proxy_async();
+        if (STAGE) bulk_wait_read();
         mbar_arrive_expect_tx(&mbar, (stage ? 0u : W_TILE_BYTES) + Z_TILE_BYTES);
-        if (!stage) tma_load_2d(sW, &mapW, x0, y0, &mbar);
+        if (!stage) tma_load_2d(sW, &mapW, x0 - PADL + a.wox, y0 - 1 + a.woy, &mbar);
         tma_load_2d(sZ, &mapZ, x0 + a.zox, y0 + a.zoy, &mbar);
       }
     } else {
+      const float inf = __int_as_float(0x7f800000);
       if (!stage) {
         for (int k = tid; k < SROWS * (SP / 4); k += FILL_THREADS) {
           const int rr = k / (SP / 4), cc = k - rr * (SP / 4);
+          const int y = y0 + rr - 1, x = x0 + 4 * cc - PADL;
           reinterpret_cast<float4 *>(sW)[k] =
-              __ldcg(reinterpret_cast<const float4 *>(a.Wp + (size_t)(y0 + rr) * a.pitch + x0) + cc);
+              a.inplace && (y < 0 || y >= a.H || x < 0 || x >= a.W)
+                  ? make_float4(inf, inf, inf, inf)
+                  : __ldcg(reinterpret_cast<const float4 *>(a.Wp + (size_t)(y + a.woy) * a.pitch + x + a.wox));
         }
       }
-      const float inf = __int_as_float(0x7f800000);
       for (int k = tid; k < TY * (TX / 4); k += FILL_THREADS) {
         const int rr = k / (TX / 4), cc = k - rr * (TX / 4);
         reinterpret_cast<float4 *>(sZ)[k] =
-            a.zext && (y0 + rr >= a.H || x0 + 4 * cc >= a.W)
+            a.inplace && (y0 + rr >= a.H || x0 + 4 * cc >= a.W)
                 ? make_float4(inf, inf, inf, inf)
                 : __ldg(reinterpret_cast<const float4 *>(a.Z + (size_t)(y0 + a.zoy + rr) * a.zpitch + x0 + a.zox) + cc);
       }
@@ -336,8 +351,8 @@
         for (; rr < SROWS; rr += RSTEP) {
           const int dy = rr == 0 ? -1 : (rr == SROWS - 1 ? 1 : 0);
           float4 v4;
-          if ((nbdone >> ((dy + 1) * 3 + dx + 1)) & 1) {
-            v4 = __ldcg(reinterpret_cast<const float4 *>(a.Wp + (size_t)(y0 + rr) * a.pitch + x0 + c4));
+          if (((nbdone >> ((dy + 1) * 3 + dx + 1)) & 1) && y0 + rr - 1 < a.H && xb < a.W) {
+            v4 = __ldcg(reinterpret_cast<const float4 *>(a.Wp + (size_t)(y0 + rr - 1 + a.woy) * a.pitch + xb + a.wox));
           } else {
             const int y = y0 + rr - 1;
             float v[4] = {inf, inf, inf, inf};
@@ -355,7 +370,7 @@
                   cc++;
                 }
                 if (x >= 0 && x < a.W)
-                  v[j] = brow || x == 0 || x == a.W - 1 ? __ldg(zrow + x) : (a.pool & 3) == 0 ? c0 : __ldg(crow + cc);
+                  v[j] = brow || x == 0 || x == a.W - 1 ? __ldcg(zrow + x) : (a.pool & 3) == 0 ? c0 : __ldg(crow + cc);
               }
             }
             v4 = make_float4(v[0], v[1], v[2], v[3]);
@@ -383,9 +398,13 @@
     if (rowout) {
       for (int k = tid; k < TY * (TX / 4); k += FILL_THREADS) {
         const int rr = k / (TX / 4), cc = k % (TX / 4);
-        if (rowout & (1 << (rr >> 2))) {
+        const int y = y0 + rr, x = x0 + 4 * cc;
+        if ((rowout & (1 << (rr >> 2))) && !(a.inplace && (y >= a.H || x >= a.W))) {
           const float4 val = *reinterpret_cast<const float4 *>(&sW[(rr + 1) * SP + PADL + 4 * cc]);
-          __stcg(reinterpret_cast<float4 *>(a.Wp + (size_t)(y0 + 1 + rr) * a.pitch + (x0 + PADL)) + cc, val);
+          __stcg(reinterpret_cast<float4 *>(a.Wp + (size_t)(y + a.woy) * a.pitch + x + a.wox), val);
+          if (STAGE && !a.use_tma)
+            __stcg(reinterpret_cast<float4 *>(a.zcopy + (size_t)y * a.W + x),
+                   *reinterpret_cast<const float4 *>(&sZ[rr * TX + 4 * cc]));
         }
       }
     }
@@ -428,6 +447,7 @@
       }
     }
   }
+  if (STAGE && a.use_tma && tid == 0) bulk_wait_all();
 }
 
 __global__ void __launch_bounds__(256) fill_admit_kernel(const FillArgs a) {
@@ -507,18 +527,17 @@
 }
 
 template <bool LIFT>
-__global__ void fill_init_kernel(const float *__restrict__ dem, float *__restrict__ Zp,
-                                 float *__restrict__ Wp, int W, int H, int pitch, int rows, FillDev *dev,
-                                 const float *__restrict__ coarse, int Wc, int pool, int yoff) {
+__global__ void fill_init_kernel(const float *dem, float *__restrict__ Zo, float *Wo, int W, int H, int pitch, int rows,
+                                 int ox, int oy, FillDev *dev, const float *__restrict__ coarse, int Wc, int pool, int yoff) {
   const int px4 = (blockIdx.x * blockDim.x + threadIdx.x) * 4;
   const float inf = __int_as_float(0x7f800000);
   float lo = inf, hi = -inf;
   for (int py = blockIdx.y; py < rows && px4 < pitch; py += gridDim.y) {
     float zv[4], wv[4];
-    const int y = py - 1;
+    const int y = py - oy;
 #pragma unroll
     for (int k = 0; k < 4; k++) {
-      const int x = px4 + k - PADL;
+      const int x = px4 + k - ox;
       float zz = inf, ww = inf;
       if (x >= 0 && x < W && y >= 0 && y < H) {
         zz = dem[(size_t)y * W + x];
@@ -533,8 +552,8 @@
       wv[k] = ww;
     }
     const size_t o = (size_t)py * pitch + px4;
-    if (Zp) *reinterpret_cast<float4 *>(Zp + o) = make_float4(zv[0], zv[1], zv[2], zv[3]);
-    *reinterpret_cast<float4 *>(Wp + o) = make_float4(wv[0], wv[1], wv[2], wv[3]);
+    *reinterpret_cast<float4 *>(Zo + o) = make_float4(zv[0], zv[1], zv[2], zv[3]);
+    *reinterpret_cast<float4 *>(Wo + o) = make_float4(wv[0], wv[1], wv[2], wv[3]);
   }
   for (int o = 16; o > 0; o >>= 1) {
     lo = fminf(lo, __shfl_xor_sync(0xffffffffu, lo, o));
@@ -552,22 +571,6 @@
     if (lo <= hi) {
       atomicMin(&dev->zmin_ord, f2ord(lo));
       atomicMax(&dev->zmax_ord, f2ord(hi));
-    }
-  }
-}
-
-__global__ void __launch_bounds__(256) fill_frame_kernel(float *__restrict__ Wp, int pitch, int rows) {
-  const int i = blockIdx.x * blockDim.x + threadIdx.x;
-  const float inf = __int_as_float(0x7f800000);
-  if (i < pitch) {
-    Wp[i] = inf;
-    Wp[(size_t)(rows - 1) * pitch + i] = inf;
-  }
-  if (i < rows) {
-#pragma unroll
-    for (int j = 0; j < PADL; j++) {
-      Wp[(size_t)i * pitch + j] = inf;
-      Wp[(size_t)i * pitch + pitch - PADL + j] = inf;
     }
   }
 }
@@ -661,10 +664,10 @@
   }
 }
 
-__global__ void __launch_bounds__(256) fill_restrict_kernel(const float *__restrict__ Wp, int pitch, int W, int H,
-                                                             float *Wc, int cpitch, int Wcw, int Hc, int k,
-                                                             const int *__restrict__ dirty, int tilesX, int *ctile_flag,
-                                                             int ctilesX) {
+__global__ void __launch_bounds__(256) fill_restrict_kernel(const float *__restrict__ Wp, int pitch, int wox, int woy, int W,
+                                                             int H, float *Wc, int cpitch, int cox, int coy, int Wcw, int Hc,
+                                                             int k, const int *__restrict__ dirty, int tilesX,
+                                                             int *ctile_flag, int ctilesX) {
   const int bx = blockIdx.x * blockDim.x + threadIdx.x;
   if (bx >= Wcw) return;
   for (int by = blockIdx.y; by < Hc; by += gridDim.y) {
@@ -672,7 +675,7 @@
     float m = -__int_as_float(0x7f800000);
     if ((k & 3) == 0 && bx * k + k <= W && by * k + k <= H) {
       for (int j = 0; j < k; j++) {
-        const float4 *row = reinterpret_cast<const float4 *>(Wp + (size_t)(by * k + j + 1) * pitch + bx * k + PADL);
+        const float4 *row = reinterpret_cast<const float4 *>(Wp + (size_t)(by * k + j + woy) * pitch + bx * k + wox);
         for (int i = 0; i < k / 4; i++) {
           const float4 q = __ldcg(row + i);
           m = fmaxf(fmaxf(m, fmaxf(q.x, q.y)), fmaxf(q.z, q.w));
@@ -684,11 +687,11 @@
         if (y >= H) break;
         for (int i = 0; i < k; i++) {
           const int x = bx * k + i;
-          if (x < W) m = fmaxf(m, __ldcg(Wp + (size_t)(y + 1) * pitch + x + PADL));
+          if (x < W) m = fmaxf(m, __ldcg(Wp + (size_t)(y + woy) * pitch + x + wox));
         }
       }
     }
-    float *o = Wc + (size_t)(by + 1) * cpitch + bx + PADL;
+    float *o = Wc + (size_t)(by + coy) * cpitch + bx + cox;
     if (m < *o && bx > 0 && by > 0 && bx < Wcw - 1 && by < Hc - 1) {
       *o = m;
       const int ty0 = (by - 1) / TY, ty1 = (by + 1) / TY, tx0 = (bx - 1) / TX, tx1 = (bx + 1) / TX;
@@ -702,7 +705,8 @@
   }
 }
 
-__global__ void __launch_bounds__(256) fill_blockmax_kernel(const float *__restrict__ Wp, int pitch, int W, int y_lo, int y_hi,
+__global__ void __launch_bounds__(256) fill_blockmax_kernel(const float *__restrict__ Wp, int pitch, int wox, int woy, int W,
+                                                             int y_lo, int y_hi,
                                                              int yoff, float *out, int Wcw, int Hc, int k,
                                                              const int *__restrict__ dirty, int tilesX) {
   const int bx = blockIdx.x * blockDim.x + threadIdx.x;
@@ -726,7 +730,7 @@
       if (y >= y_hi) break;
       for (int i = 0; i < k; i++) {
         const int x = bx * k + i;
-        if (x < W) m = fmaxf(m, __ldcg(Wp + (size_t)(y + 1) * pitch + x + PADL));
+        if (x < W) m = fmaxf(m, __ldcg(Wp + (size_t)(y + woy) * pitch + x + wox));
       }
     }
     float *o = out + (size_t)by * Wcw + bx;
@@ -734,7 +738,8 @@
   }
 }
 
-__global__ void __launch_bounds__(256) fill_prolong_kernel(float *Wp, int pitch, int W, int H, const float *__restrict__ Wc,
+__global__ void __launch_bounds__(256) fill_prolong_kernel(float *Wp, int pitch, int wox, int woy, int W, int H,
+                                                            const float *__restrict__ Wc,
                                                             int cpitch, int coff_x, int coff_y, int k, int *tile_flag,
                                                             int tilesX, int yoff, const int *__restrict__ cdirty,
                                                             int ctilesX) {
@@ -753,8 +758,8 @@
   for (int g = threadIdx.x; g < TX * TY / 4; g += blockDim.x) {
     const int ly = g / (TX / 4), lx4 = (g - ly * (TX / 4)) * 4;
     const int y = y0 + ly;
-    if (y < 1 || y >= H - 1) continue;
-    float4 *wp4 = reinterpret_cast<float4 *>(Wp + (size_t)(y + 1) * pitch + x0 + lx4 + PADL);
+    if (y < 1 || y >= H - 1 || x0 + lx4 >= W) continue;
+    float4 *wp4 = reinterpret_cast<float4 *>(Wp + (size_t)(y + woy) * pitch + x0 + lx4 + wox);
     const float4 w4 = *wp4;
     float wv[4] = {w4.x, w4.y, w4.z, w4.w};
     const float *crow = Wc + (size_t)((y + yoff) / k + coff_y) * cpitch + coff_x;
@@ -794,20 +799,20 @@
 }
 
 __global__ void __launch_bounds__(256) fill_finish_x4_kernel(const float *__restrict__ Wp, float *__restrict__ out, int W,
-                                                              int H, int pitch) {
+                                                              int H, int pitch, int wox, int woy) {
   const int x4 = (blockIdx.x * blockDim.x + threadIdx.x) * 4;
   if (x4 >= W) return;
   for (int y = blockIdx.y; y < H; y += gridDim.y) {
-    const float4 v = __ldcs(reinterpret_cast<const float4 *>(Wp + (size_t)(y + 1) * pitch + x4 + PADL));
+    const float4 v = __ldcs(reinterpret_cast<const float4 *>(Wp + (size_t)(y + woy) * pitch + x4 + wox));
     __stcs(reinterpret_cast<float4 *>(out + (size_t)y * W + x4), v);
   }
 }
 
 __global__ void fill_finish_kernel(const float *__restrict__ Wp, float *__restrict__ out, int W, int H,
-                                   int pitch) {
+                                   int pitch, int wox, int woy) {
   const int x = blockIdx.x * blockDim.x + threadIdx.x;
   if (x >= W) return;
-  for (int y = blockIdx.y; y < H; y += gridDim.y) out[(size_t)y * W + x] = Wp[(size_t)(y + 1) * pitch + x + PADL];
+  for (int y = blockIdx.y; y < H; y += gridDim.y) out[(size_t)y * W + x] = Wp[(size_t)(y + woy) * pitch + x + wox];
 }
 
 typedef CUresult (*EncodeTiledFn)(CUtensorMap *, CUtensorMapDataType, cuuint32_t, void *, const cuuint64_t *,
@@ -864,12 +869,27 @@
   bool still_active = false;
   int64_t sched_round = 0;
 
-  const float *zext = nullptr;
+  float *Wb = nullptr;
+  int wpitch = 0, wox = 0, woy = 0;
+  bool inplace = false;
+  DevBuf<float> Zc;
   const float *stage_coarse = nullptr;
   int stage_wc = 0, stage_k = 1, stage_yoff = 0;
+  CUtensorMap mapZstage;
+
+  void use_padded_layout(size_t np) {
+    inplace = false;
+    Zc.reset();
+    Zp.alloc(np);
+    Wp.alloc(np);
+    Wb = Wp.p;
+    wpitch = pitch;
+    wox = PADL;
+    woy = 1;
+  }
 
   void begin(const float *d_dem, int w, int h, const float *d_coarse = nullptr, int coarse_w = 0, int coarse_k = 0,
-             int coarse_yoff = 0, bool dem_stays = false) {
+             int coarse_yoff = 0, bool in_place = false) {
     Ctx &c = ctx();
     W = w;
     H = h;
@@ -878,14 +898,21 @@
     pitch = tilesX * TX + 2 * PADL;
     rows = tilesY * TY + 2;
     const size_t np = (size_t)pitch * rows;
-    zext = dem_stays && c.params.fill_external_z != 0 && (w & 3) == 0 && ((uintptr_t)d_dem & 15) == 0 ? d_dem : nullptr;
-    stage_coarse = zext && d_coarse ? d_coarse : nullptr;
+    if (in_place && c.params.fill_external_z != 0 && (w & 3) == 0 && ((uintptr_t)d_dem & 15) == 0) {
+      inplace = true;
+      Zp.reset();
+      Wp.reset();
+      Zc.alloc((size_t)w * h);
+      Wb = const_cast<float *>(d_dem);
+      wpitch = w;
+      wox = woy = 0;
+    } else {
+      use_padded_layout(np);
+    }
+    stage_coarse = inplace && d_coarse ? d_coarse : nullptr;
     stage_wc = coarse_w;
     stage_k = coarse_k;
     stage_yoff = coarse_yoff;
-    if (zext) Zp.reset();
-    else Zp.alloc(np);
-    Wp.alloc(np);
     const size_t nt = (size_t)tilesX * tilesY;
     list0.alloc(nt);
     list1.alloc(nt);
@@ -911,18 +938,23 @@
     {
       const int n2 = (int)(2 * nt);
       fill_i32_kernel<<<(n2 + 255) / 256, 256, 0, c.stream>>>(keys.p, ORD_POS_INF, n2);
+      count_launch();
       dim3 blk(128), grd((pitch / 4 + 127) / 128, rows < 2048 ? rows : 2048);
       if (stage_coarse) {
-        const int n = pitch > rows ? pitch : rows;
-        fill_frame_kernel<<<(n + 255) / 256, 256, 0, c.stream>>>(Wp.p, pitch, rows);
+      } else if (inplace) {
+        dim3 grdc((W / 4 + 127) / 128, H < 2048 ? H : 2048);
+        fill_init_kernel<false><<<grdc, blk, 0, c.stream>>>(d_dem, Zc.p, Wb, W, H, W, H, 0, 0, dev.p, nullptr, 0, 1, 0);
+        count_launch();
       } else if (d_coarse) {
-        fill_init_kernel<true><<<grd, blk, 0, c.stream>>>(d_dem, Zp.p, Wp.p, W, H, pitch, rows, dev.p, d_coarse, coarse_w, coarse_k,
-                                                         coarse_yoff);
+        fill_init_kernel<true><<<grd, blk, 0, c.stream>>>(d_dem, Zp.p, Wp.p, W, H, pitch, rows, PADL, 1, dev.p, d_coarse,
+                                                         coarse_w, coarse_k, coarse_yoff);
+        count_launch();
       } else {
-        fill_init_kernel<false><<<grd, blk, 0, c.stream>>>(d_dem, Zp.p, Wp.p, W, H, pitch, rows, dev.p, nullptr, 0, 1, 0);
+        fill_init_kernel<false><<<grd, blk, 0, c.stream>>>(d_dem, Zp.p, Wp.p, W, H, pitch, rows, PADL, 1, dev.p, nullptr, 0, 1,
+                                                          0);
+        count_launch();
       }
       RDB_CK(cudaGetLastError());
-      count_launch(2);
       zmin = zmax = 0.f;
       if (!d_coarse) {
         FillDev *hd = (FillDev *)c.pinned;
@@ -944,8 +976,8 @@
           RDB_CK(cudaMemsetAsync(hist.p, 0, HIST_BINS * sizeof(unsigned int), c.stream));
           const int stride = rows > 4096 ? 16 : (rows > 512 ? 4 : 1);
           const int nb = (rows - 2 + stride - 1) / stride;
-          if (zext)
-            fill_hist_kernel<<<nb, 256, 0, c.stream>>>(zext, W, W, H, stride, zmin, 1.0f / (zmax - zmin), hist.p);
+          if (inplace)
+            fill_hist_kernel<<<nb, 256, 0, c.stream>>>(Zc.p, W, W, H, stride, zmin, 1.0f / (zmax - zmin), hist.p);
           else
             fill_hist_kernel<<<nb, 256, 0, c.stream>>>(Zp.p + pitch, pitch, pitch, rows - 1, stride, zmin, 1.0f / (zmax - zmin),
                                                        hist.p);
@@ -967,8 +999,14 @@
         }
       }
     }
-    mapW = make_map(Wp.p, pitch, rows, SP, SROWS);
-    mapZ = zext ? make_map(const_cast<float *>(zext), W, H, TX, TY) : make_map(Zp.p, pitch, rows, TX, TY);
+    if (inplace) {
+      mapW = make_map(Wb, W, H, SP, SROWS);
+      mapZ = make_map(Zc.p, W, H, TX, TY);
+      if (stage_coarse) mapZstage = make_map(Wb, W, H, TX, TY);
+    } else {
+      mapW = make_map(Wp.p, pitch, rows, SP, SROWS);
+      mapZ = make_map(Zp.p, pitch, rows, TX, TY);
+    }
     int per_sm = 0;
     RDB_CK(cudaOccupancyMaxActiveBlocksPerMultiprocessor(&per_sm, fill_sweep_kernel<0>, FILL_THREADS, 0));
     if (per_sm < 1) per_sm = 1;
@@ -991,9 +1029,7 @@
     tilesY = (h + TY - 1) / TY;
     pitch = tilesX * TX + 2 * PADL;
     rows = tilesY * TY + 2;
-    const size_t np = (size_t)pitch * rows;
-    Zp.alloc(np);
-    Wp.alloc(np);
+    use_padded_layout((size_t)pitch * rows);
     const size_t nt = (size_t)tilesX * tilesY;
     list0.alloc(nt);
     list1.alloc(nt);
@@ -1041,10 +1077,10 @@
     Ctx &c = ctx();
     FillArgs a;
     memset(&a, 0, sizeof(a));
-    if (zext) {
-      a.Z = zext;
+    if (inplace) {
+      a.Z = Zc.p;
       a.zpitch = W;
-      a.zext = 1;
+      a.inplace = 1;
     } else {
       a.Z = Zp.p;
       a.zpitch = pitch;
@@ -1055,8 +1091,10 @@
     a.pool = stage_k;
     a.yoff = stage_yoff;
     a.staged = staged.p;
-    a.Wp = Wp.p;
-    a.pitch = pitch;
+    a.Wp = Wb;
+    a.pitch = wpitch;
+    a.wox = wox;
+    a.woy = woy;
     a.W = W;
     a.H = H;
     a.tilesX = tilesX;
@@ -1095,11 +1133,14 @@
       }
       sched_round++;
       a.coarse = round == 1 ? stage_coarse : nullptr;
-      if (step_mode) fill_sweep_kernel<1><<<grid, FILL_THREADS, 0, c.stream>>>(mapW, mapZ, a);
-      else if (a.coarse && topo4) fill_sweep_kernel<0, true, true><<<grid, FILL_THREADS, 0, c.stream>>>(mapW, mapZ, a);
-      else if (a.coarse) fill_sweep_kernel<0, false, true><<<grid, FILL_THREADS, 0, c.stream>>>(mapW, mapZ, a);
-      else if (topo4) fill_sweep_kernel<0, true><<<grid, FILL_THREADS, 0, c.stream>>>(mapW, mapZ, a);
-      else fill_sweep_kernel<0><<<grid, FILL_THREADS, 0, c.stream>>>(mapW, mapZ, a);
+      a.Z = a.coarse ? Wb : (inplace ? Zc.p : Zp.p);
+      a.zcopy = a.coarse ? Zc.p : nullptr;
+      const CUtensorMap &mz = a.coarse ? mapZstage : mapZ;
+      if (step_mode) fill_sweep_kernel<1><<<grid, FILL_THREADS, 0, c.stream>>>(mapW, mz, mapZ, a);
+      else if (a.coarse && topo4) fill_sweep_kernel<0, true, true><<<grid, FILL_THREADS, 0, c.stream>>>(mapW, mz, mapZ, a);
+      else if (a.coarse) fill_sweep_kernel<0, false, true><<<grid, FILL_THREADS, 0, c.stream>>>(mapW, mz, mapZ, a);
+      else if (topo4) fill_sweep_kernel<0, true><<<grid, FILL_THREADS, 0, c.stream>>>(mapW, mz, mapZ, a);
+      else fill_sweep_kernel<0><<<grid, FILL_THREADS, 0, c.stream>>>(mapW, mz, mapZ, a);
       round++;
     }
     if (timed) RDB_CK(cudaEventRecord(c.evk1, c.stream));
@@ -1184,8 +1225,8 @@
     cs.clear_flags();
     const bool selective = dirty.p && TX % k == 0 && TY % k == 0;
     dim3 blk(256), grd((unsigned)((cs.W + 255) / 256), (unsigned)(cs.H < 4096 ? cs.H : 4096));
-    fill_restrict_kernel<<<grd, blk, 0, c.stream>>>(Wp.p, pitch, W, H, cs.Wp.p, cs.pitch, cs.W, cs.H, k,
-                                                    selective ? dirty.p : nullptr, tilesX, cs.tflag.p, cs.tilesX);
+    fill_restrict_kernel<<<grd, blk, 0, c.stream>>>(Wb, wpitch, wox, woy, W, H, cs.Wb, cs.wpitch, cs.wox, cs.woy, cs.W, cs.H,
+                                                    k, selective ? dirty.p : nullptr, tilesX, cs.tflag.p, cs.tilesX);
     RDB_CK(cudaGetLastError());
     count_launch();
     cs.seed_from_flags();
@@ -1195,7 +1236,8 @@
     Ctx &c = ctx();
     dim3 blk(256), grd((unsigned)((wc + 255) / 256), (unsigned)((y_hi - y_lo) / k + 2 < 4096 ? (y_hi - y_lo) / k + 2 : 4096));
     const bool sel = selective && dirty.p && TX % k == 0;
-    fill_blockmax_kernel<<<grd, blk, 0, c.stream>>>(Wp.p, pitch, W, y_lo, y_hi, yoff, d_out, wc, hc, k, sel ? dirty.p : nullptr, tilesX);
+    fill_blockmax_kernel<<<grd, blk, 0, c.stream>>>(Wb, wpitch, wox, woy, W, y_lo, y_hi, yoff, d_out, wc, hc, k,
+                                                    sel ? dirty.p : nullptr, tilesX);
     RDB_CK(cudaGetLastError());
     count_launch();
     if (sel) clear_dirty();
@@ -1205,14 +1247,14 @@
     Ctx &c = ctx();
     clear_flags();
     const int nt = tilesX * tilesY;
-    fill_prolong_kernel<<<nt, 256, 0, c.stream>>>(Wp.p, pitch, W, H, d_wc, cpitch, coff_x, coff_y, k, tflag.p, tilesX, yoff,
-                                                  cdirty, ctilesX);
+    fill_prolong_kernel<<<nt, 256, 0, c.stream>>>(Wb, wpitch, wox, woy, W, H, d_wc, cpitch, coff_x, coff_y, k, tflag.p, tilesX,
+                                                  yoff, cdirty, ctilesX);
     RDB_CK(cudaGetLastError());
     count_launch();
     seed_from_flags(d_count);
   }
   void prolong_from_level(FillState &cs, int k, int yoff = 0, int *d_count = nullptr) {
-    prolong_from(cs.Wp.p, cs.pitch, PADL, 1, k, yoff, cs.dirty.p, cs.tilesX, d_count);
+    prolong_from(cs.Wb, cs.wpitch, cs.wox, cs.woy, k, yoff, cs.dirty.p, cs.tilesX, d_count);
     cs.clear_dirty();
   }
   void ghost_update(int y, const float *d_row, int *d_lowered) {
@@ -1226,7 +1268,7 @@
 
   void read_row(int y, float *d_row) {
     if (y < 0 || y >= H) fail("fill_read_row: row %d out of range", y);
-    RDB_CK(cudaMemcpyAsync(d_row, Wp.p + (size_t)(y + 1) * pitch + PADL, (size_t)W * 4,
+    RDB_CK(cudaMemcpyAsync(d_row, Wb + (size_t)(y + woy) * wpitch + wox, (size_t)W * 4,
                            cudaMemcpyDeviceToDevice, ctx().stream));
   }
 
@@ -1263,12 +1305,13 @@
 
   void finish(float *d_out) {
     Ctx &c = ctx();
+    if (d_out == Wb) return;
     if ((W & 3) == 0 && ((uintptr_t)d_out & 15) == 0) {
       dim3 blk(256), grd((W / 4 + 255) / 256, H < 4096 ? H : 4096);
-      fill_finish_x4_kernel<<<grd, blk, 0, c.stream>>>(Wp.p, d_out, W, H, pitch);
+      fill_finish_x4_kernel<<<grd, blk, 0, c.stream>>>(Wb, d_out, W, H, wpitch, wox, woy);
     } else {
       dim3 blk(256), grd((W + 255) / 256, H < 32768 ? H : 32768);
-      fill_finish_kernel<<<grd, blk, 0, c.stream>>>(Wp.p, d_out, W, H, pitch);
+      fill_finish_kernel<<<grd, blk, 0, c.stream>>>(Wb, d_out, W, H, wpitch, wox, woy);
     }
     RDB_CK(cudaGetLastError());
     count_launch();
diff --git a/richdem_b200/csrc/fill_relax_body.inc b/richdem_b200/csrc/fill_relax_body.inc
--- a/richdem_b200/csrc/fill_relax_body.inc
+++ b/richdem_b200/csrc/fill_relax_body.inc
@@ -25,14 +25,26 @@
     if (a.use_tma) {
       mbar_wait(&mbar, phase);
       phase ^= 1;
-      if (a.zext && (x0 + TX > a.W || y0 + TY > a.H)) {
-        for (int k = tid; k < TX * TY; k += FILL_THREADS) {
-          const int rr = k / TX, cc = k - rr * TX;
-          if (y0 + rr >= a.H || x0 + cc >= a.W) sZ[k] = __int_as_float(0x7f800000);
+      if (a.inplace) {
+        const float inf = __int_as_float(0x7f800000);
+        if (!STAGE && (x0 == 0 || y0 == 0 || x0 + TX + PADL > a.W || y0 + TY + 1 > a.H)) {
+          for (int k = tid; k < SROWS * SP; k += FILL_THREADS) {
+            const int rr = k / SP, cc = k - rr * SP;
+            const int y = y0 + rr - 1, x = x0 + cc - PADL;
+            if (y < 0 || y >= a.H || x < 0 || x >= a.W) sW[k] = inf;
+          }
+        }
+        if (x0 + TX > a.W || y0 + TY > a.H) {
+          for (int k = tid; k < TX * TY; k += FILL_THREADS) {
+            const int rr = k / TX, cc = k - rr * TX;
+            if (y0 + rr >= a.H || x0 + cc >= a.W) sZ[k] = inf;
+          }
+          if (STAGE) fence_proxy_async();
         }
       }
     }
     __syncthreads();
+    if (STAGE && a.use_tma && tid == 0) tma_store_2d(&mapZout, x0, y0, sZ);
     if constexpr (STAGE && DRAIN_SWEEPS) fill_drain_sweeps<TOPO4>(sW, sZ, y0, a.H, &sFlags, &sKey);
 
     int f = 0;
```

Measured after the change: 21350, median of 6. 1.05x the previous value.
